# OCSYT/SoftwareRenderer

Measured on AMD Instinct MI355X. Metric: Mfragments/s (depth-tested + textured fragments, whole frame), higher is better.
Workload: dtype f32; 1 GPU; cfg3: 4096x4096, 1000000 triangles in 16 u16 meshes, 2048^2 RGBA8 nearest texture, program Dust2LambertFog, Back/LessEqual/Alpha; pipelining=1, parallelism=1 GPU

## Files before the change

### softwarerenderer_amd/csrc/swr_api.hip

```cpp
#include <hip/hip_runtime.h>
#include <hip/hiprtc.h>
#include <dlfcn.h>

#include <algorithm>
#include <cstddef>
#include <cmath>
#include <cstdio>
#include <cstdlib>
#include <cstring>
#include <map>
#include <memory>
#include <mutex>
#include <string>
#include <vector>
#if defined(SWR_RTC_FLAGS)
#include "swr_rtc_sources.inc"
#endif

#include "swr.h"
#include "swr_device.h"
#include "swr_geometry.hip.h"
#include "swr_binning.hip.h"
#include "swr_raster.hip.h"
#include "swr_raster_c.hip.h"
#include "swr_cull.hip.h"

using namespace swr;

#define SWR_STR2(x) #x
#define SWR_STR(x) SWR_STR2(x)

#include "swr_host.h"
#include "swr_rtc.h"
#include "swr_flush.h"

namespace {
int launch_flatten(swr_context* c, float* d_rgb, size_t n) {
    const int blocks = (int)std::min<size_t>((n + 255) / 256, 2048 * 8);
    hipLaunchKernelGGL(k_flatten_rgb, dim3(blocks), dim3(256), 0, c->stream, (const float4*)c->color, d_rgb, n);
    SWR_HIP(c, hipGetLastError());
    return SWR_OK;
}

int flatten_device(swr_context* c, float* d_rgb, bool validate) {
    if (!d_rgb) return fail(c, SWR_ERR_INVALID_ARG, "d_rgb is null");
    int rc = flush_locked(c); if (rc) return rc;
    const size_t n = band_pixels(c);
    if (!n) return SWR_OK;
    if (validate && (rc = sync_locked(c))) return rc;
    return launch_flatten(c, d_rgb, n);
}

int planes_transfer(swr_context* c, float* color, float* depth, bool to_host) {
    int rc = flush_and_sync_locked(c); if (rc) return rc;
    const size_t n = band_pixels(c);
    const hipMemcpyKind kind = to_host ? hipMemcpyDeviceToHost : hipMemcpyHostToDevice;
    if (n && color) SWR_HIP(c, hipMemcpyAsync(to_host ? (void*)color : c->color, to_host ? (void*)c->color : color, n * 16, kind, c->stream));
    if (n && depth) SWR_HIP(c, hipMemcpyAsync(to_host ? depth : c->depth, to_host ? c->depth : depth, n * 4, kind, c->stream));
    return sync_locked(c);
}

int pixel_transfer(swr_context* c, int x, int y, void* plane, size_t bytes, void* host, bool to_host) {
    if (x < 0 || x >= c->W || band_local_pixel_row(c, y) < 0) return SWR_OK;
    int rc = flush_and_sync_locked(c); if (rc) return rc;
    void* dev = static_cast<char*>(plane) + ((size_t)band_local_pixel_row(c, y) * c->W + x) * bytes;
    if (to_host) SWR_HIP(c, hipMemcpyAsync(host, dev, bytes, hipMemcpyDeviceToHost, c->stream));
    else SWR_HIP(c, hipMemcpyAsync(dev, host, bytes, hipMemcpyHostToDevice, c->stream));
    return sync_locked(c);
}
}

extern "C" {

int swr_abi_version(void) { return SWR_ABI_VERSION; }

#ifndef SWR_BUILD_HIPCC
#define SWR_BUILD_HIPCC "unknown"
#endif
#ifndef SWR_BUILD_SRC_SHA
#define SWR_BUILD_SRC_SHA "unknown"
#endif
#ifndef SWR_BUILD_EXTRA
#define SWR_BUILD_EXTRA ""
#endif
const char* swr_build_info(void) {
    return "hipcc=" SWR_BUILD_HIPCC "; csrc_sha256=" SWR_BUILD_SRC_SHA "; fma=" SWR_STR(SWR_NUMERICS_FMA) "; dot=" SWR_STR(SWR_DOT_PAIRWISE) "; extra=" SWR_BUILD_EXTRA;
}

int swr_numerics_mode(int* fma, int* dot_order) {
    if (!fma || !dot_order) return SWR_ERR_INVALID_ARG;
    *fma = SWR_NUMERICS_FMA; *dot_order = SWR_DOT_PAIRWISE;
    return SWR_OK;
}

int swr_set_transform_fma(swr_context* c, int transform_fused, int transform_normal_fused) {
    if (!c) return SWR_ERR_INVALID_ARG;
    std::lock_guard<std::mutex> lock_(c->mu);
    c->nm_flags = (transform_fused ? SWR_NM_TRANSFORM_FMA : 0u) | (transform_normal_fused ? SWR_NM_TRANSFORM_NORMAL_FMA : 0u);
    return SWR_OK;
}

int swr_get_transform_fma(swr_context* c, int* transform_fused, int* transform_normal_fused) {
    if (!c || !transform_fused || !transform_normal_fused) return SWR_ERR_INVALID_ARG;
    std::lock_guard<std::mutex> lock_(c->mu);
    *transform_fused = (c->nm_flags & SWR_NM_TRANSFORM_FMA) ? 1 : 0;
    *transform_normal_fused = (c->nm_flags & SWR_NM_TRANSFORM_NORMAL_FMA) ? 1 : 0;
    return SWR_OK;
}

const char* swr_last_error(const swr_context* ctx) { return ctx ? ctx->err.c_str() : g_create_error.c_str(); }

int swr_create(int device_id, swr_context** out) {
    if (!out) { g_create_error = "out is null"; return SWR_ERR_INVALID_ARG; }
    *out = nullptr;
    int n = 0;
    hipError_t e = hipGetDeviceCount(&n);
    if (e != hipSuccess || n <= 0) {
        g_create_error = std::string("no HIP device available: ") + hipGetErrorString(e) + " (this backend has no CPU fallback)";
        return SWR_ERR_NO_DEVICE;
    }
    if (device_id < 0 || device_id >= n) { g_create_error = "device id out of range"; return SWR_ERR_INVALID_ARG; }
    if ((e = hipSetDevice(device_id)) != hipSuccess) { g_create_error = hipGetErrorString(e); return SWR_ERR_HIP; }
    hipDeviceProp_t prop;
    if ((e = hipGetDeviceProperties(&prop, device_id)) != hipSuccess) { g_create_error = hipGetErrorString(e); return SWR_ERR_HIP; }
    if (strncmp(prop.gcnArchName, "gfx950", 6) != 0) {
        g_create_error = std::string("device is ") + prop.gcnArchName + "; libswr_hip.so carries gfx950 code objects only";
        return SWR_ERR_NO_DEVICE;
    }
    swr_context* c = new swr_context();
    c->device = device_id;
    snprintf(c->dev_name, sizeof c->dev_name, "%s (%s)", prop.name, prop.gcnArchName);
    if ((e = hipStreamCreateWithFlags(&c->own_stream, hipStreamNonBlocking)) != hipSuccess) {
        g_create_error = hipGetErrorString(e); delete c; return SWR_ERR_HIP;
    }
    c->stream = c->own_stream;
    if (ensure_front_stream(c)) { g_create_error = c->err; (void)hipStreamDestroy(c->own_stream); delete c; return SWR_ERR_HIP; }
    { const char* sf = getenv("SWR_SYNC_FLUSH"); c->sync_flush = sf && sf[0] == '1'; }
#ifdef SWR_TEST_HOOKS
    { const char* df = getenv("SWR_DEBUG_FILL_CAPACITY"); c->debug_fill_capacity = df ? (uint32_t)strtoul(df, nullptr, 10) : 0u; }
#endif
    int rc = ensure(c, c->d_counters, 65 * sizeof(Counters));
    if (!rc) rc = ensure(c, c->d_ctrl, 64);
    if (!rc && hipHostMalloc((void**)&c->host_poison, 64, hipHostMallocDefault) != hipSuccess) rc = SWR_ERR_OOM;
    if (!rc) { memset(c->host_poison, 0, 64); rc = reset_ctrl(c); }
    if (!rc) rc = ensure(c, c->d_total, 256 + 4096 * 8);
    if (!rc && hipMemsetAsync(c->d_total.p, 0, 256 + 4096 * 8, c->stream) != hipSuccess) rc = SWR_ERR_HIP;
    if (!rc && hipMemsetAsync(c->d_counters.p, 0, 65 * sizeof(Counters), c->stream) != hipSuccess) rc = SWR_ERR_HIP;
    if (rc) { g_create_error = c->err; swr_destroy(c); return rc; }
    *out = c;
    return SWR_OK;
}

void swr_destroy(swr_context* c) {
    if (!c) return;
    (void)hipSetDevice(c->device);
    (void)hipStreamSynchronize(c->stream);
    if (c->front_stream) (void)hipStreamSynchronize(c->front_stream);
    for (auto& d : c->draws) if (d.mesh && d.mesh->transient) c->garbage.push_back(d.mesh);
    for (auto& b : c->inflight) retire_batch(c, b);
    c->inflight.clear();
    collect_spans(c);
    free_garbage(c);
    c->draws.clear();
    c->progs.clear();
    for (swr_mesh* m : c->mesh_pool) destroy_mesh(m);
    c->mesh_pool.clear();
    for (hipEvent_t e : c->event_pool) (void)hipEventDestroy(e);
    for (auto& fs : c->slots) { if (fs.host) (void)hipHostFree(fs.host); if (fs.done) (void)hipEventDestroy(fs.done); }
    if (c->host_poison) (void)hipHostFree(c->host_poison);
    if (c->copy_stream) { (void)hipStreamSynchronize(c->copy_stream); (void)hipStreamDestroy(c->copy_stream); }
    for (int i = 0; i < 2; ++i) {
        if (c->present_flat[i]) (void)hipEventDestroy(c->present_flat[i]);
        if (c->present_done[i]) (void)hipEventDestroy(c->present_done[i]);
        release(c->present_buf[i]);
    }
    DevBuf* bufs[] = { &c->own_color, &c->own_depth, &c->d_slot_tb, &c->d_want, &c->d_ctrl, &c->d_pair_tile, &c->d_tile_list, &c->d_tile_stats,
                       &c->d_counters, &c->d_total, &c->d_scratch };
    for (DevBuf* b : bufs) release(*b);
    for (auto& s : c->sets) {
        DevBuf* sb[] = { &s.d_upload, &s.d_vout, &s.d_vnorm, &s.d_recs, &s.d_masks, &s.d_pcounts, &s.d_pair_refs, &s.d_tile_count, &s.d_tile_start, &s.d_order };
        for (DevBuf* b : sb) release(*b);
        if (s.front_done) (void)hipEventDestroy(s.front_done);
        if (s.raster_done) (void)hipEventDestroy(s.raster_done);
    }
    if (c->front_stream) (void)hipStreamDestroy(c->front_stream);
    if (c->f_tail_ev) (void)hipEventDestroy(c->f_tail_ev);
    if (c->r_front_ev) (void)hipEventDestroy(c->r_front_ev);
    if (c->own_stream) (void)hipStreamDestroy(c->own_stream);
    delete c;
}

#define SWR_ENTER(c)                                   \
    if (!(c)) return SWR_ERR_INVALID_ARG;              \
    std::lock_guard<std::mutex> lock_((c)->mu);        \
    (void)hipSetDevice((c)->device)

int swr_resize(swr_context* c, int width, int height) {
    SWR_ENTER(c);
    if (width > 65535 || height > 65535) return fail(c, SWR_ERR_INVALID_ARG, "render target larger than 65535");
    if (c->geometry_applied && width == c->W && height == c->H) return SWR_OK;
    int rc = flush_and_sync_locked(c); if (rc) return rc;
    c->W = width; c->H = height;
    c->geometry_applied = true;
    return apply_geometry(c);
}

int swr_set_band(swr_context* c, int first_tile_row, int n_tile_rows) {
    SWR_ENTER(c);
    const bool want_band = !(first_tile_row < 0 || n_tile_rows < 0);
    if (c->il_k == 0 && want_band == c->band_set && (!want_band || (first_tile_row == c->band_first && n_tile_rows == c->band_count)))
        return SWR_OK;
    int rc = flush_and_sync_locked(c); if (rc) return rc;
    c->il_k = 0; c->il_world = 1; c->il_rank = 0;
    c->band_set = want_band;
    if (want_band) { c->band_first = first_tile_row; c->band_count = n_tile_rows; }
    return apply_geometry(c);
}

int swr_set_band_interleaved(swr_context* c, int rank, int world, int stripe_tile_rows) {
    SWR_ENTER(c);
    if (world < 1 || rank < 0 || rank >= world || stripe_tile_rows < 1) return fail(c, SWR_ERR_INVALID_ARG, "bad interleaved band arguments");
    if (c->il_k == stripe_tile_rows && c->il_world == world && c->il_rank == rank) return SWR_OK;
    int rc = flush_and_sync_locked(c); if (rc) return rc;
    c->band_set = false;
    c->il_k = stripe_tile_rows; c->il_world = world; c->il_rank = rank;
    return apply_geometry(c);
}

int swr_bind_framebuffer(swr_context* c, void* color, void* depth) {
    SWR_ENTER(c);
    if ((color == nullptr) != (depth == nullptr)) return fail(c, SWR_ERR_INVALID_ARG, "bind both colour and depth, or neither");
    int rc = flush_locked(c); if (rc) return rc;
    if (!color && (rc = sync_locked(c))) return rc;
    c->ext_color = color; c->ext_depth = depth;
    return apply_geometry(c);
}

int swr_set_stream(swr_context* c, void* s) {
    SWR_ENTER(c);
    int rc = flush_and_sync_locked(c); if (rc) return rc;
    c->stream = s ? (hipStream_t)s : c->own_stream;
    return SWR_OK;
}

int swr_clear_color(swr_context* c, const float rgba[4]) {
    SWR_ENTER(c);
    if (!rgba) return fail(c, SWR_ERR_INVALID_ARG, "rgba is null");
    if (!c->draws.empty()) { int rc = flush_locked(c); if (rc) return rc; }
    memcpy(c->clear_rgba, rgba, 16);
    c->pend_clear_color = true;
    return SWR_OK;
}

int swr_clear_depth(swr_context* c) {
    SWR_ENTER(c);
    if (!c->draws.empty()) { int rc = flush_locked(c); if (rc) return rc; }
    c->pend_clear_depth = true;
    return SWR_OK;
}

int swr_flush(swr_context* c) { SWR_ENTER(c); return flush_locked(c); }

int swr_set_pipelining(swr_context* c, int mode) {
    SWR_ENTER(c);
    if (mode < 0 || mode > 2) return fail(c, SWR_ERR_INVALID_ARG, "pipelining mode must be 0 (off), 1 (every batch) or 2 (only frames of up to 2^15 tiles or batches of up to 2^17 triangles)");
    if (mode == c->pipelining) return SWR_OK;
    int rc = flush_and_sync_locked(c); if (rc) return rc;
    c->pipelining = mode;
    return ensure_front_stream(c);
}

int swr_get_pipelining(swr_context* c, int* mode) { SWR_ENTER(c); if (!mode) return SWR_ERR_INVALID_ARG; *mode = c->pipelining; return SWR_OK; }

int swr_sync(swr_context* c) {
    SWR_ENTER(c);
    return flush_and_sync_locked(c);
}

int swr_readback(swr_context* c, float* color, float* depth) { SWR_ENTER(c); return planes_transfer(c, color, depth, true); }

int swr_readback_rgb(swr_context* c, float* rgb) {
    SWR_ENTER(c);
    if (!rgb) return fail(c, SWR_ERR_INVALID_ARG, "rgb is null");
    int rc = flush_and_sync_locked(c); if (rc) return rc;
    size_t n = band_pixels(c);
    if (!n) return SWR_OK;
    if ((rc = ensure(c, c->d_scratch, n * 12))) return rc;
    if ((rc = launch_flatten(c, c->d_scratch.as<float>(), n))) return rc;
    SWR_HIP(c, hipMemcpyAsync(rgb, c->d_scratch.p, n * 12, hipMemcpyDeviceToHost, c->stream));
    return sync_locked(c);
}

int swr_present_rgb_async(swr_context* c, float* rgb, uint64_t* ticket) {
    SWR_ENTER(c);
    if (!rgb || !ticket) return fail(c, SWR_ERR_INVALID_ARG, "rgb or ticket is null");
    int rc = flush_locked(c); if (rc) return rc;
    const size_t n = band_pixels(c);
    const int slot = (int)(c->next_ticket & 1ull);
    if (!c->copy_stream) SWR_HIP(c, hipStreamCreateWithFlags(&c->copy_stream, hipStreamNonBlocking));
    for (int i = 0; i < 2; ++i) {
        if (!c->present_flat[i]) SWR_HIP(c, hipEventCreateWithFlags(&c->present_flat[i], hipEventDisableTiming));
        if (!c->present_done[i]) SWR_HIP(c, hipEventCreateWithFlags(&c->present_done[i], hipEventDisableTiming));
    }
    if (c->present_ticket[slot]) {
        SWR_HIP(c, hipEventSynchronize(c->present_done[slot]));
        bool stale = false;
        if ((rc = present_is_stale(c, slot, stale))) return rc;
        if (stale) c->stale_dropped[slot] = c->present_ticket[slot];
        c->present_ticket[slot] = 0;
    }
    if (n) {
        if (c->present_buf[slot].cap < n * 12) {
            SWR_HIP(c, hipStreamSynchronize(c->copy_stream));
            if ((rc = ensure(c, c->present_buf[slot], n * 12))) return rc;
        }
        if ((rc = launch_flatten(c, c->present_buf[slot].as<float>(), n))) return rc;
    }
    SWR_HIP(c, hipEventRecord(c->present_flat[slot], c->stream));
    SWR_HIP(c, hipStreamWaitEvent(c->copy_stream, c->present_flat[slot], 0));
    if (n) SWR_HIP(c, hipMemcpyAsync(rgb, c->present_buf[slot].p, n * 12, hipMemcpyDeviceToHost, c->copy_stream));
    SWR_HIP(c, hipEventRecord(c->present_done[slot], c->copy_stream));
    c->present_ticket[slot] = ++c->next_ticket;
    c->present_seq[slot] = c->next_seq - 1u;
    *ticket = c->present_ticket[slot];
    return SWR_OK;
}

int swr_present_wait(swr_context* c, uint64_t ticket) {
    SWR_ENTER(c);
    int slot = -1;
    for (int i = 0; i < 2; ++i) if (c->present_ticket[i] == ticket && ticket) slot = i;
    if (slot < 0) {
        if (!ticket || ticket > c->next_ticket) return fail(c, SWR_ERR_INVALID_ARG, "unknown present ticket");
        for (int i = 0; i < 2; ++i)
            if (c->stale_dropped[i] == ticket) { c->stale_dropped[i] = 0; return SWR_STALE; }
        return SWR_OK;
    }
    SWR_HIP(c, hipEventSynchronize(c->present_done[slot]));
    c->present_ticket[slot] = 0;
    bool stale = false;
    int rc = present_is_stale(c, slot, stale); if (rc) return rc;
    if (stale) {
        rc = sync_locked(c);
        return rc ? rc : SWR_STALE;
    }
    const uint32_t upto = c->present_seq[slot];
    size_t k = 0;
    while (k < c->inflight.size() && c->inflight[k].seq <= upto) { retire_batch(c, c->inflight[k], true); ++k; }
    c->inflight.erase(c->inflight.begin(), c->inflight.begin() + (std::ptrdiff_t)k);
    return SWR_OK;
}

int swr_host_register(swr_context* c, void* ptr, size_t bytes) {
    SWR_ENTER(c);
    if (!ptr || !bytes) return fail(c, SWR_ERR_INVALID_ARG, "null or empty host buffer");
    SWR_HIP(c, hipHostRegister(ptr, bytes, hipHostRegisterDefault));
    return SWR_OK;
}

int swr_host_unregister(swr_context* c, void* ptr) {
    SWR_ENTER(c);
    if (!ptr) return fail(c, SWR_ERR_INVALID_ARG, "null host buffer");
    int rc = flush_and_sync_locked(c); if (rc) return rc;
    SWR_HIP(c, hipHostUnregister(ptr));
    return SWR_OK;
}

int swr_flatten_rgb_device(swr_context* c, float* d_rgb) { SWR_ENTER(c); return flatten_device(c, d_rgb, true); }
int swr_flatten_rgb_device_async(swr_context* c, float* d_rgb) { SWR_ENTER(c); return flatten_device(c, d_rgb, false); }

int swr_replay_count(swr_context* c, uint64_t* out) { SWR_ENTER(c); if (!out) return SWR_ERR_INVALID_ARG; *out = c->replays; return SWR_OK; }
int swr_sync_count(swr_context* c, uint64_t* out) { SWR_ENTER(c); if (!out) return SWR_ERR_INVALID_ARG; *out = c->host_syncs; return SWR_OK; }

int swr_upload(swr_context* c, const float* color, const float* depth) {
    SWR_ENTER(c);
    return planes_transfer(c, const_cast<float*>(color), const_cast<float*>(depth), false);
}

int swr_color_device_ptr(swr_context* c, void** out) { SWR_ENTER(c); if (!out) return SWR_ERR_INVALID_ARG; *out = c->color; return SWR_OK; }
int swr_depth_device_ptr(swr_context* c, void** out) { SWR_ENTER(c); if (!out) return SWR_ERR_INVALID_ARG; *out = c->depth; return SWR_OK; }

int swr_get_pixel(swr_context* c, int x, int y, float rgba[4]) {
    SWR_ENTER(c);
    if (!rgba) return SWR_ERR_INVALID_ARG;
    rgba[0] = rgba[1] = rgba[2] = rgba[3] = 0.0f;
    return pixel_transfer(c, x, y, c->color, 16, rgba, true);
}
int swr_set_pixel(swr_context* c, int x, int y, const float rgba[4]) {
    SWR_ENTER(c);
    if (!rgba) return SWR_ERR_INVALID_ARG;
    return pixel_transfer(c, x, y, c->color, 16, const_cast<float*>(rgba), false);
}
int swr_get_depth(swr_context* c, int x, int y, float* d) {
    SWR_ENTER(c);
    if (!d) return SWR_ERR_INVALID_ARG;
    *d = SWR_FLOAT_MINVALUE;
    return pixel_transfer(c, x, y, c->depth, 4, d, true);
}
int swr_set_depth(swr_context* c, int x, int y, float d) {
    SWR_ENTER(c);
    return pixel_transfer(c, x, y, c->depth, 4, &d, false);
}

int swr_texture_create(swr_context* c, const uint8_t* rgba8, int w, int h, swr_texture** out) {
    SWR_ENTER(c);
    if (!rgba8 || w <= 0 || h <= 0 || !out) return fail(c, SWR_ERR_INVALID_ARG, "bad texture arguments");
    if ((uint64_t)w * (uint64_t)h >= (1ull << 30)) return fail(c, SWR_ERR_UNSUPPORTED, "textures of 2^30 texels or more are not supported (32-bit texel index)");
    swr_texture* t = new swr_texture();
    t->w = w; t->h = h;
    hipError_t e = hipMalloc((void**)&t->d_rgba, (size_t)w * h * 4);
    if (e == hipSuccess) e = hipMemcpyAsync(t->d_rgba, rgba8, (size_t)w * h * 4, hipMemcpyHostToDevice, c->stream);
    if (e != hipSuccess) {
        if (t->d_rgba) (void)hipFree(t->d_rgba);
        delete t;
        c->err = std::string("texture upload failed: ") + hipGetErrorString(e);
        return e == hipErrorOutOfMemory ? SWR_ERR_OOM : SWR_ERR_HIP;
    }
    *out = t;
    return SWR_OK;
}

int swr_texture_set_filter(swr_context* c, swr_texture* t, int bilinear) {
    SWR_ENTER(c);
    if (!t) return fail(c, SWR_ERR_INVALID_ARG, "texture is null");
    t->bilinear = bilinear != 0;
    if (t->bilinear && !t->d_blocked && (t->w & 3) == 0 && (t->h & 3) == 0) {
        SWR_HIP(c, hipMalloc((void**)&t->d_blocked, (size_t)t->w * t->h * 4));
        const int blocks = (int)std::min<size_t>(((size_t)t->w * t->h + 255) / 256, 2048 * 8);
        hipLaunchKernelGGL(k_block_texture, dim3(blocks), dim3(256), 0, c->stream, (const uint32_t*)t->d_rgba, (uint32_t*)t->d_blocked, t->w, t->h);
        SWR_HIP(c, hipGetLastError());
    }
    return SWR_OK;
}

int swr_texture_destroy(swr_context* c, swr_texture* t) {
    SWR_ENTER(c);
    if (!t) return SWR_OK;
    int rc = flush_and_sync_locked(c); if (rc) return rc;
    if (t->d_rgba) (void)hipFree(t->d_rgba);
    if (t->d_blocked) (void)hipFree(t->d_blocked);
    delete t;
    return SWR_OK;
}

int swr_texture_sample(swr_context* c, const swr_texture* t, const float* uv, int n, float* out) {
    SWR_ENTER(c);
    if (!t || !uv || !out || n < 0) return fail(c, SWR_ERR_INVALID_ARG, "bad texture_sample arguments");
    if (n == 0) return SWR_OK;
    const size_t off_out = ((size_t)n * 8 + 15) & ~(size_t)15;
    int rc = ensure(c, c->d_scratch, off_out + (size_t)n * 16);
    if (rc) return rc;
    float2* d_uv = c->d_scratch.as<float2>();
    float4* d_out = reinterpret_cast<float4*>(reinterpret_cast<char*>(c->d_scratch.p) + off_out);
    SWR_HIP(c, hipMemcpyAsync(d_uv, uv, (size_t)n * 8, hipMemcpyHostToDevice, c->stream));
    hipLaunchKernelGGL(k_texture_sample, dim3((n + 255) / 256), dim3(256), 0, c->stream, t->d_rgba, t->w, t->h, d_uv, n, d_out);
    SWR_HIP(c, hipGetLastError());
    SWR_HIP(c, hipMemcpyAsync(out, d_out, (size_t)n * 16, hipMemcpyDeviceToHost, c->stream));
    return sync_locked(c);
}

int swr_mesh_create(swr_context* c, const swr_vertex* v, int nv, const uint16_t* idx, int ni, swr_mesh** out) { SWR_ENTER(c); return make_mesh(c, v, nv, idx, ni, false, out); }

int swr_mesh_destroy(swr_context* c, swr_mesh* m) {
    SWR_ENTER(c);
    if (!m) return SWR_OK;
    int rc = flush_and_sync_locked(c); if (rc) return rc;
    destroy_mesh(m);
    return SWR_OK;
}

int swr_set_state(swr_context* c, float near_clip, float far_clip, int debug_mode) {
    SWR_ENTER(c);
    if (debug_mode != SWR_DEBUG_NONE && debug_mode != SWR_DEBUG_WIREFRAME) return fail(c, SWR_ERR_INVALID_ARG, "bad debug mode");
    if (!c->draws.empty() && (near_clip != c->near_clip || debug_mode != c->debug_mode)) {
        int rc = flush_locked(c); if (rc) return rc;
    }
    c->near_clip = near_clip; c->far_clip = far_clip; c->debug_mode = debug_mode;
    return SWR_OK;
}

int swr_initialize_tile_locks(swr_context* c, int width, int height) {
    SWR_ENTER(c);
    if (width <= 0 || height <= 0)
        return fail(c, SWR_ERR_INVALID_ARG, "Width and height must be positive non-zero values.");
    return SWR_OK;
}

int swr_render_mesh(swr_context* c, const swr_mesh* mesh, const float model[16], const float view[16], const float proj[16],
                    int program, const swr_uniforms* u, const swr_texture* tex, int cull, int depth_test, int blend) {
    SWR_ENTER(c); return record_draw(c, const_cast<swr_mesh*>(mesh), model, view, proj, program, u, tex, cull, depth_test, blend);
}

int swr_render_mesh_culled(swr_context* c, const swr_mesh* mesh, const float model[16], const float view[16], const float proj[16],
                           int program, const swr_uniforms* u, const swr_texture* tex, int cull, int depth_test, int blend) {
    SWR_ENTER(c); return record_draw(c, const_cast<swr_mesh*>(mesh), model, view, proj, program, u, tex, cull, depth_test, blend, true);
}

int swr_mesh_bounds(swr_context* c, const swr_mesh* mesh, float center_radius[4]) {
    SWR_ENTER(c);
    if (!mesh || !center_radius) return fail(c, SWR_ERR_INVALID_ARG, "bad mesh_bounds arguments");
    int rc = ensure_bounds(c, const_cast<swr_mesh*>(mesh));
    if (rc) return rc;
    SWR_HIP(c, hipMemcpyAsync(center_radius, mesh->d_bounds, 16, hipMemcpyDeviceToHost, use_front_stream(c)));
    SWR_HIP(c, hipStreamSynchronize(use_front_stream(c)));
    return SWR_OK;
}

int swr_is_sphere_in_frustum(swr_context* c, const float center_radius[4], const float model[16], const float view[16],
                             const float proj[16], int* inside) {
    SWR_ENTER(c);
    if (!center_radius || !model || !view || !proj || !inside) return fail(c, SWR_ERR_INVALID_ARG, "bad is_sphere_in_frustum arguments");
    int rc = ensure(c, c->d_scratch, 256);
    if (rc) return rc;
    float h[48];
    memcpy(h, model, 64); memcpy(h + 16, view, 64); memcpy(h + 32, proj, 64);
    char* base = reinterpret_cast<char*>(c->d_scratch.p);
    SWR_HIP(c, hipMemcpyAsync(base, h, sizeof h, hipMemcpyHostToDevice, c->stream));
    hipLaunchKernelGGL(k_frustum_test, dim3(1), dim3(64), 0, c->stream,
                       make_float4(center_radius[0], center_radius[1], center_radius[2], center_radius[3]),
                       (const float*)base, (uint32_t*)(base + 192), c->nm_flags);
    SWR_HIP(c, hipGetLastError());
    uint32_t r = 0;
    SWR_HIP(c, hipMemcpyAsync(&r, base + 192, 4, hipMemcpyDeviceToHost, c->stream));
    SWR_HIP(c, hipStreamSynchronize(c->stream));
    *inside = (int)r;
    return SWR_OK;
}

int swr_program_validate(const char* src, char* log, int log_len) { return swr_program_validate_vf(nullptr, src, log, log_len); }

int swr_program_validate_vf(const char* vertex_src, const char* src, char* log, int log_len) {
    if (!src) return SWR_ERR_INVALID_ARG;
    std::shared_ptr<const RtcCode> code;
    std::string msg;
    const int rc = rtc_compile(vertex_src, src, code, msg);
    if (log && log_len > 0) {
        const size_t n = std::min(msg.size(), (size_t)log_len - 1);
        memcpy(log, msg.data(), n); log[n] = '\0';
    }
    return rc;
}

int swr_program_create(swr_context* c, const char* src, int* program_id) { return swr_program_create_vf(c, nullptr, src, program_id); }

int swr_program_create_vf(swr_context* c, const char* vertex_src, const char* src, int* program_id) {
    SWR_ENTER(c);
    if (!src || !program_id) return fail(c, SWR_ERR_INVALID_ARG, "null argument to swr_program_create");
    std::shared_ptr<const RtcCode> code;
    std::string log;
    const int rc = rtc_compile(vertex_src, src, code, log);
    if (rc) { c->err = log; return rc; }
    auto p = std::make_shared<UserProg>();
    SWR_HIP(c, hipModuleLoadData(&p->mod, code->code.data()));
    for (int k = 0; k < 2; ++k) SWR_HIP(c, hipModuleGetFunction(&p->fn[k], p->mod, code->names[k].c_str()));
    if (code->has_vertex) {
        SWR_HIP(c, hipModuleGetFunction(&p->vertex_fn, p->mod, code->names[2].c_str()));
        SWR_HIP(c, hipModuleGetFunction(&p->setup_fn, p->mod, code->names[3].c_str()));
    }
    const int id = c->next_prog++;
    c->progs[id] = std::move(p);
    *program_id = id;
    return SWR_OK;
}

int swr_program_destroy(swr_context* c, int program_id) {
    SWR_ENTER(c);
    auto it = c->progs.find(program_id);
    if (it == c->progs.end()) return fail(c, SWR_ERR_INVALID_ARG, "unknown or destroyed user program id");
    c->progs.erase(it);
    return SWR_OK;
}

int swr_program_set_constants(swr_context* c, int program_id, const float* values, int n) {
    SWR_ENTER(c);
    auto it = c->progs.find(program_id);
    if (it == c->progs.end()) return fail(c, SWR_ERR_INVALID_ARG, "unknown or destroyed user program id");
    if (n < 0 || n > 64 || (n > 0 && !values)) return fail(c, SWR_ERR_INVALID_ARG, "between 0 and 64 constants");
    float* k = it->second->constants;
    for (int i = 0; i < 64; ++i) k[i] = i < n ? values[i] : 0.0f;
    return SWR_OK;
}

int swr_render_mesh_arrays(swr_context* c, const swr_vertex* v, int nv, const uint16_t* idx, int ni,
                           const float model[16], const float view[16], const float proj[16],
                           int program, const swr_uniforms* u, const swr_texture* tex, int cull, int depth_test, int blend) {
    SWR_ENTER(c);
    if (c->W <= 0 || c->H <= 0) return SWR_OK;
    swr_mesh* m = nullptr;
    int rc = make_mesh(c, v, nv, idx, ni, true, &m);
    if (rc) return rc;
    rc = record_draw(c, m, model, view, proj, program, u, tex, cull, depth_test, blend);
    if (rc || c->draws.empty() || c->draws.back().mesh != m) c->garbage.push_back(m);
    return rc;
}

int swr_interpolate(swr_context* c, const float* verts60, const float* w, int n, int interpolate, float* out) {
    SWR_ENTER(c);
    if (!verts60 || !w || !out || n < 0) return fail(c, SWR_ERR_INVALID_ARG, "bad interpolate arguments");
    if (n == 0) return SWR_OK;
    const size_t off_w = 256, off_o = 256 + (((size_t)n * 12 + 15) & ~(size_t)15);
    int rc = ensure(c, c->d_scratch, off_o + (size_t)n * 96);
    if (rc) return rc;
    char* base = reinterpret_cast<char*>(c->d_scratch.p);
    SWR_HIP(c, hipMemcpyAsync(base, verts60, 240, hipMemcpyHostToDevice, c->stream));
    SWR_HIP(c, hipMemcpyAsync(base + off_w, w, (size_t)n * 12, hipMemcpyHostToDevice, c->stream));
    hipLaunchKernelGGL(k_interpolate, dim3((n + 255) / 256), dim3(256), 0, c->stream,
                       (const float*)base, (const float*)(base + off_w), n, interpolate, (float*)(base + off_o));
    SWR_HIP(c, hipGetLastError());
    SWR_HIP(c, hipMemcpyAsync(out, base + off_o, (size_t)n * 96, hipMemcpyDeviceToHost, c->stream));
    return sync_locked(c);
}

int swr_get_stats(swr_context* c, swr_stats* out) {
    SWR_ENTER(c);
    if (!out) return SWR_ERR_INVALID_ARG;
    int rc = flush_and_sync_locked(c); if (rc) return rc;
    Counters host[65];
    unsigned long long frag[3] = { 0, 0, 0 };
    if (c->tile_stats_tiles) {
        unsigned long long* d3 = c->d_total.as<unsigned long long>() + 1;
        hipLaunchKernelGGL(k_reduce_tile_stats, dim3(1), dim3(1024), 0, c->stream, c->d_tile_stats.as<uint32_t>(),
                           (uint32_t)c->tile_stats_tiles, d3, 0);
        SWR_HIP(c, hipGetLastError());
        SWR_HIP(c, hipMemcpyAsync(frag, d3, 24, hipMemcpyDeviceToHost, c->stream));
    }
    unsigned long long carry[3] = { 0, 0, 0 };
    SWR_HIP(c, hipMemcpyAsync(carry, c->d_total.as<unsigned long long>() + 4, 24, hipMemcpyDeviceToHost, c->stream));
    SWR_HIP(c, hipMemcpyAsync(host, c->d_counters.p, sizeof host, hipMemcpyDeviceToHost, c->stream));
    if ((rc = sync_locked(c))) return rc;
    swr_stats s = {};
    for (int i = 0; i < 65; ++i) {
        s.triangles_in += host[i].triangles_in; s.triangles_setup += host[i].triangles_setup;
        s.triangles_clipped += host[i].triangles_clipped; s.tile_pairs += host[i].tile_pairs;
    }
    s.fragments_tested = frag[0] + carry[0]; s.fragments_shaded = frag[1] + carry[1]; s.fragments_written = frag[2] + carry[2];
    s.tile_pairs += c->host_tile_pairs;
    s.flushes = c->totals.flushes;
    *out = s;
    return SWR_OK;
}

int swr_reset_stats(swr_context* c) {
    SWR_ENTER(c);
    int rc = flush_locked(c); if (rc) return rc;
    SWR_HIP(c, hipMemsetAsync(c->d_counters.p, 0, 65 * sizeof(Counters), c->stream));
    if (c->tile_stats_tiles) SWR_HIP(c, hipMemsetAsync(c->d_tile_stats.p, 0, c->tile_stats_tiles * 12, c->stream));
    SWR_HIP(c, hipMemsetAsync(c->d_total.as<unsigned long long>() + 4, 0, 24, c->stream));
    c->totals = {}; c->host_tile_pairs = 0;
    return sync_locked(c);
}

int swr_profile_enable(swr_context* c, int on) {
    SWR_ENTER(c);
    int rc = flush_and_sync_locked(c); if (rc) return rc;
    c->profiling = on < 0 ? 0 : (on > 3 ? 1 : on);
    c->raster_span_no = 0;
    return SWR_OK;
}
int swr_profile_get(swr_context* c, swr_profile* out) {
    SWR_ENTER(c);
    if (!out) return SWR_ERR_INVALID_ARG;
    int rc = flush_and_sync_locked(c); if (rc) return rc;
    c->prof.flushes = c->totals.flushes;
    *out = c->prof;
    return SWR_OK;
}
int swr_profile_reset(swr_context* c) {
    SWR_ENTER(c);
    int rc = flush_and_sync_locked(c); if (rc) return rc;
    c->prof = {};
    c->raster_samples.clear();
    return SWR_OK;
}
int swr_profile_raster_samples(swr_context* c, float* out_ms, int capacity, int* n) {
    SWR_ENTER(c);
    if (!n || capacity < 0 || (capacity > 0 && !out_ms)) return SWR_ERR_INVALID_ARG;
    int rc = flush_and_sync_locked(c); if (rc) return rc;
    const int have = (int)c->raster_samples.size();
    for (int i = 0; i < std::min(have, capacity); ++i) out_ms[i] = c->raster_samples[(size_t)i];
    *n = have;
    return SWR_OK;
}

int swr_debug_counters(swr_context* c, uint64_t out[8]) {
    SWR_ENTER(c);
    if (!out) return SWR_ERR_INVALID_ARG;
    int rc = flush_and_sync_locked(c); if (rc) return rc;
    SWR_HIP(c, hipMemcpyAsync(out, c->d_total.as<unsigned long long>() + 8, 64, hipMemcpyDeviceToHost, c->stream));
    if ((rc = sync_locked(c))) return rc;
    SWR_HIP(c, hipMemsetAsync(c->d_total.as<unsigned long long>() + 8, 0, 64, c->stream));
    return SWR_OK;
}

int swr_selftest_division(swr_context* c, uint64_t samples, uint64_t seed, uint64_t out[8]) {
    SWR_ENTER(c);
    if (!out) return SWR_ERR_INVALID_ARG;
    int rc = flush_locked(c); if (rc) return rc;
    if ((rc = ensure(c, c->d_scratch, 64))) return rc;
    SWR_HIP(c, hipMemsetAsync(c->d_scratch.p, 0, 64, c->stream));
    const int iters = 1024;
    const uint64_t per_block = 256ull * (uint64_t)iters;
    const unsigned blocks = (unsigned)std::min<uint64_t>((samples + per_block - 1) / per_block, 1u << 20);
    if (blocks) hipLaunchKernelGGL(k_selftest_division, dim3(blocks), dim3(256), 0, c->stream, (unsigned long long)seed, iters,
                                   c->d_scratch.as<unsigned long long>());
    SWR_HIP(c, hipGetLastError());
    hipLaunchKernelGGL(k_selftest_recip, dim3(16384), dim3(256), 0, c->stream, c->d_scratch.as<unsigned long long>());
    SWR_HIP(c, hipGetLastError());
    SWR_HIP(c, hipMemcpyAsync(out, c->d_scratch.p, 64, hipMemcpyDeviceToHost, c->stream));
    return sync_locked(c);
}

int swr_device_name(swr_context* c, char* buf, int buflen) {
    SWR_ENTER(c);
    if (!buf || buflen <= 0) return SWR_ERR_INVALID_ARG;
    snprintf(buf, (size_t)buflen, "%s", c->dev_name);
    return SWR_OK;
}

}
```

### softwarerenderer_amd/csrc/swr_binning.hip.h

```cpp
#pragma once
#include "swr_device.h"

#define SWR_ORDER_BUCKETS 256

namespace swr {

struct BinArgs {
    const unsigned long long* __restrict__ slot_tb;
    const TriRec* __restrict__ recs;
    uint32_t odd_base;
    uint32_t slot_lo, slot_hi;
    uint32_t spt;
    int tiles_x;
    BandMap band;
    int width, height;
    uint32_t* __restrict__ tile_count;
    const uint32_t* __restrict__ tile_start;
    uint32_t* __restrict__ tile_list;
    uint32_t list_capacity;
    Counters* __restrict__ counters;
    Ctrl* __restrict__ ctrl;
    uint32_t seq;
    uint32_t replayable;
    const unsigned long long* __restrict__ total;
    const uint8_t* __restrict__ want;
    uint32_t tpw;
    uint32_t bin_blocks;
    int order_tiles_y;
    const uint8_t* __restrict__ tile_bucket;
    const uint32_t* __restrict__ order_hist;
    uint32_t* __restrict__ order_cursor;
    uint4* __restrict__ tile_order;
};


__device__ __forceinline__ void bin_overflow(const BinArgs& a) {
    a.counters->overflow = 1u;
    if (a.ctrl->host_flag) __hip_atomic_store(a.ctrl->host_flag + 1, 1u, __ATOMIC_RELAXED, __HIP_MEMORY_SCOPE_SYSTEM);
    if (a.replayable) {
        atomicMin(&a.ctrl->first_bad, a.seq);
        atomicMax(&a.ctrl->need, 2ull * (unsigned long long)a.list_capacity + 4096ull);
        __hip_atomic_store(&a.ctrl->poison, 1u, __ATOMIC_RELAXED, __HIP_MEMORY_SCOPE_AGENT);
        if (a.ctrl->host_flag) __hip_atomic_store(a.ctrl->host_flag, 1u, __ATOMIC_RELAXED, __HIP_MEMORY_SCOPE_SYSTEM);
    }
}

__device__ __forceinline__ uint32_t order_bucket(uint32_t w) {
    if (w == 0u) return 0u;
    const int e = 31 - __clz((int)w);
    const uint32_t m = e >= 3 ? ((w >> (e - 3)) & 7u) : ((w << (3 - e)) & 7u);
    return min((uint32_t)(e * 8) + m + 1u, (uint32_t)SWR_ORDER_BUCKETS - 1u);
}
__device__ __forceinline__ uint32_t tile_weight(uint32_t frags, uint32_t pairs) { return frags + 16u * pairs; }

__device__ __forceinline__ uint32_t order_tile_of_thread(uint32_t block, int tiles_x, int tiles_y) {
    const int sbx = (tiles_x + 15) >> 4;
    const int bx = (int)(block % (uint32_t)sbx), by = (int)(block / (uint32_t)sbx);
    const int t = threadIdx.x, q = t >> 6, w = t & 63;
    const int tx = bx * 16 + (q & 1) * 8 + (w & 7), ty = by * 16 + (q >> 1) * 8 + (w >> 3);
    return (tx < tiles_x && ty < tiles_y) ? (uint32_t)(ty * tiles_x + tx) : 0xffffffffu;
}
__host__ __device__ inline uint32_t order_blocks(int tiles_x, int tiles_y) { return (uint32_t)(((tiles_x + 15) / 16) * ((tiles_y + 15) / 16)); }

__device__ __forceinline__ void tile_place_block(const BinArgs& a, uint32_t block, uint32_t* s_suf, uint32_t* s_cnt) {
    const uint32_t t = threadIdx.x;
    s_suf[t] = a.order_hist[t];
    s_cnt[t] = 0u;
    __syncthreads();
    for (uint32_t off = 1; off < (uint32_t)SWR_ORDER_BUCKETS; off <<= 1) {
        const uint32_t v = t + off < (uint32_t)SWR_ORDER_BUCKETS ? s_suf[t + off] : 0u;
        __syncthreads();
        s_suf[t] += v;
        __syncthreads();
    }
    const uint32_t i = order_tile_of_thread(block, a.tiles_x, a.order_tiles_y);
    uint32_t b = 0, rank = 0;
    if (i != 0xffffffffu) {
        b = a.tile_bucket[i];
        rank = atomicAdd(&s_cnt[b], 1u);
    }
    __syncthreads();
    const uint32_t mine = s_cnt[t];
    __syncthreads();
    if (mine) s_cnt[t] = (s_suf[t] - a.order_hist[t]) + atomicAdd(&a.order_cursor[t], mine);
    __syncthreads();
    if (i != 0xffffffffu) {
        const uint32_t n_tiles = (uint32_t)(a.tiles_x * a.order_tiles_y);
        const uint32_t st = a.tile_start[i];
        const unsigned long long nxt = i + 1u < n_tiles ? (unsigned long long)a.tile_start[i + 1u] : *a.total;
        a.tile_order[s_cnt[b] + rank] = make_uint4(i, st, (uint32_t)(nxt - st), 0u);
    }
}

struct SlotData {
    int tminx, tminy, nx, ny;
    float sx[3], sy[3];
    int minX, maxX, minY, maxY;
    bool is_line;
};
__device__ __forceinline__ SlotData slot_load(const BinArgs& a, uint32_t slot, unsigned long long tb) {
    SlotData s;
    s.sx[0] = s.sx[1] = s.sx[2] = s.sy[0] = s.sy[1] = s.sy[2] = 0.f;
    s.minX = s.minY = 0; s.maxX = s.maxY = -1; s.is_line = false;
    SlotTiles st;
    slot_tiles(a.band, tb, st);
    s.tminx = st.tminx; s.tminy = st.tminy; s.nx = st.nx; s.ny = st.ny;
    if (s.nx * s.ny > SWR_SMALL_TILES) {
        const float4* __restrict__ rq = reinterpret_cast<const float4*>(a.recs + rec_index(slot, a.odd_base));
        const float4 r0 = rq[0], r1 = rq[1], r3 = rq[3];
        s.sx[0] = r0.x; s.sx[1] = r0.y; s.sx[2] = r0.z; s.sy[0] = r0.w; s.sy[1] = r1.x; s.sy[2] = r1.y;
        const uint32_t bbx = __float_as_uint(r3.y), bby = __float_as_uint(r3.z);
        s.minX = (int)(bbx & 0xffffu); s.maxX = (int)(bbx >> 16); s.minY = (int)(bby & 0xffffu); s.maxY = (int)(bby >> 16);
        s.is_line = (__float_as_uint(r3.w) & SWR_FLAG_LINE) != 0u;
    }
    return s;
}

template <bool FILL>
__device__ __forceinline__ void bin_big(const BinArgs& a, const SlotData& sd, uint32_t slot, bool big) {
    const int lane = threadIdx.x & 63;
    const int nt = sd.nx * sd.ny;
    unsigned long long med = __ballot(big && nt <= 64);
    while (med) {
        bool want[4];
        uint32_t tile[4], sslot[4], base[4];
#pragma unroll
        for (int j = 0; j < 4; ++j) {
            want[j] = false; tile[j] = 0u; sslot[j] = 0u; base[j] = 0u;
            if (med) {
                const int src = __ffsll((long long)med) - 1;
                med &= med - 1;
                const int s_tminx = __shfl(sd.tminx, src), s_tminy = __shfl(sd.tminy, src);
                const int s_nx = __shfl(sd.nx, src), s_nt = __shfl(nt, src);
                sslot[j] = (uint32_t)__shfl((int)slot, src);
                float bsx[3], bsy[3];
#pragma unroll
                for (int k = 0; k < 3; ++k) { bsx[k] = __shfl(sd.sx[k], src); bsy[k] = __shfl(sd.sy[k], src); }
                const int bminX = __shfl(sd.minX, src), bmaxX = __shfl(sd.maxX, src), bminY = __shfl(sd.minY, src), bmaxY = __shfl(sd.maxY, src);
                const bool b_line = __shfl((int)sd.is_line, src) != 0;
                if (lane < s_nt) {
                    const int ty = s_tminy + lane / s_nx, tx = s_tminx + lane % s_nx;
                    want[j] = band_local_row(a.band, ty) >= 0 && pair_may_cover(bsx, bsy, bminX, bmaxX, bminY, bmaxY, tx, ty, a.width, a.height, b_line);
                    tile[j] = (uint32_t)(band_local_row(a.band, ty) * a.tiles_x + tx);
                }
                if (want[j]) {
                    if (FILL) base[j] = atomicAdd(&a.tile_count[tile[j]], 1u);
                    else atomicAdd(&a.tile_count[tile[j]], 1u);
                }
            }
        }
        if (FILL) {
#pragma unroll
            for (int j = 0; j < 4; ++j) {
                if (want[j]) {
                    const uint32_t at = a.tile_start[tile[j]] + base[j];
                    if (at < a.list_capacity) a.tile_list[at] = sslot[j];
                    else bin_overflow(a);
                }
            }
        }
    }
    unsigned long long m = __ballot(big && nt > 64);
    while (m) {
        const int src = __ffsll((long long)m) - 1;
        m &= m - 1;
        const int s_tminx = __shfl(sd.tminx, src), s_tminy = __shfl(sd.tminy, src);
        const int s_nx = __shfl(sd.nx, src), s_nt = __shfl(nt, src);
        const uint32_t s_slot = (uint32_t)__shfl((int)slot, src);
        float bsx[3], bsy[3];
#pragma unroll
        for (int k = 0; k < 3; ++k) { bsx[k] = __shfl(sd.sx[k], src); bsy[k] = __shfl(sd.sy[k], src); }
        const int bminX = __shfl(sd.minX, src), bmaxX = __shfl(sd.maxX, src), bminY = __shfl(sd.minY, src), bmaxY = __shfl(sd.maxY, src);
        const bool b_line = __shfl((int)sd.is_line, src) != 0;
        for (int i0 = 0; i0 < s_nt; i0 += 64) {
            const int i = i0 + lane;
            bool want = i < s_nt;
            int ty = 0, tx = 0;
            if (want) {
                ty = s_tminy + i / s_nx; tx = s_tminx + i % s_nx;
                want = band_local_row(a.band, ty) >= 0 && pair_may_cover(bsx, bsy, bminX, bmaxX, bminY, bmaxY, tx, ty, a.width, a.height, b_line);
            }
            if (want) {
                const uint32_t tile = (uint32_t)(band_local_row(a.band, ty) * a.tiles_x + tx);
                if (FILL) {
                    const uint32_t at = a.tile_start[tile] + atomicAdd(&a.tile_count[tile], 1u);
                    if (at < a.list_capacity) a.tile_list[at] = s_slot;
                    else bin_overflow(a);
                } else {
                    atomicAdd(&a.tile_count[tile], 1u);
                }
            }
        }
    }
}

#define SWR_BIN_TABLE_LOG2 8
#define SWR_BIN_TABLE (1 << SWR_BIN_TABLE_LOG2)
template <bool FILL>
__device__ __forceinline__ void bin_block_slots(const BinArgs& a, uint32_t slot, unsigned long long tb, uint32_t want_in, uint32_t* s_key, uint32_t* s_val) {
    const SlotData sd = slot_load(a, slot, tb);
    const int nt = sd.nx * sd.ny;
    const bool big = nt > SWR_SMALL_TILES;
    const int nt_small = big ? 0 : nt;
    if (!__syncthreads_or(nt != 0)) return;
    for (int e = threadIdx.x; e < SWR_BIN_TABLE; e += 256) { s_key[e] = 0u; s_val[e] = 0u; }
    __syncthreads();
    uint32_t packed[SWR_SMALL_TILES];
    SlotTiles st; st.tminx = sd.tminx; st.tminy = sd.tminy; st.nx = sd.nx; st.ny = sd.ny;
    SmallTileWalk w(st);
    const uint32_t wmask = nt_small ? want_in : 0u;
#pragma unroll
    for (int i = 0; i < SWR_SMALL_TILES; ++i) {
        packed[i] = 0u;
        if (i < nt_small) {
            if ((wmask >> i) & 1u) {
                const uint32_t tile = (uint32_t)(band_local_row(a.band, w.ty) * a.tiles_x + w.tx);
                uint32_t e = (tile * 0x9E3779B1u) >> (32 - SWR_BIN_TABLE_LOG2);
                bool placed = false;
                for (int probe = 0; probe < 16; ++probe) {
                    const uint32_t prev = atomicCAS(&s_key[e], 0u, tile + 1u);
                    if (prev == 0u || prev == tile + 1u) { placed = true; break; }
                    e = (e + 1u) & (SWR_BIN_TABLE - 1u);
                }
                if (placed) {
                    const uint32_t rank = atomicAdd(&s_val[e], 1u);
                    packed[i] = e | (rank << 12) | 0x80000000u;
                } else if (FILL) {
                    const uint32_t at = a.tile_start[tile] + atomicAdd(&a.tile_count[tile], 1u);
                    if (at < a.list_capacity) a.tile_list[at] = slot;
                    else bin_overflow(a);
                } else {
                    atomicAdd(&a.tile_count[tile], 1u);
                }
            }
            w.next();
        }
    }
    __syncthreads();
    for (int e = threadIdx.x; e < SWR_BIN_TABLE; e += 256) {
        const uint32_t key = s_key[e];
        if (key) {
            const uint32_t tile = key - 1u, n = s_val[e];
            if (FILL) s_val[e] = a.tile_start[tile] + atomicAdd(&a.tile_count[tile], n);
            else atomicAdd(&a.tile_count[tile], n);
        }
    }
    if (FILL) {
        __syncthreads();
#pragma unroll
        for (int i = 0; i < SWR_SMALL_TILES; ++i) {
            if (packed[i] & 0x80000000u) {
                const uint32_t at = s_val[packed[i] & 0xfffu] + ((packed[i] >> 12) & 0x7ffffu);
                if (at < a.list_capacity) a.tile_list[at] = slot;
                else bin_overflow(a);
            }
        }
    }
    bin_big<FILL>(a, sd, slot, big);
}

template <bool FILL>
__global__ __launch_bounds__(256) void k_bin(BinArgs a) {
    SWR_FRONT_ENTER();
    __shared__ uint32_t s_key[SWR_BIN_TABLE];
    __shared__ uint32_t s_val[SWR_BIN_TABLE];
    if (FILL && batch_poisoned(a.ctrl, a.seq)) return;
    if (FILL && blockIdx.x >= a.bin_blocks) {
        static_assert(SWR_BIN_TABLE >= SWR_ORDER_BUCKETS, "tile_place_block borrows the hash table's LDS");
        tile_place_block(a, blockIdx.x - a.bin_blocks, s_key, s_val);
        return;
    }
    const uint32_t wave_id = (blockIdx.x * 256u + threadIdx.x) >> 6, lane_id = threadIdx.x & 63u;
    const bool has_tri = lane_id < a.tpw;
    const uint32_t first = a.slot_lo + (wave_id * a.tpw + lane_id) * a.spt;
    auto in_round = [&](uint32_t si) { return has_tri && si < a.spt && first + si < a.slot_hi; };
    auto tb_of = [&](uint32_t si) { return in_round(si) ? a.slot_tb[first + si] : SWR_TB_INVALID; };
    auto want_of = [&](uint32_t si) { return in_round(si) ? (uint32_t)a.want[first + si] : 0u; };
    unsigned long long tb = tb_of(0);
    uint32_t wm = want_of(0);
    for (uint32_t si = 0; si < a.spt; ++si) {
        const unsigned long long tb_next = tb_of(si + 1);
        const uint32_t wm_next = want_of(si + 1);
        bin_block_slots<FILL>(a, first + si, tb, wm, s_key, s_val);
        tb = tb_next; wm = wm_next;
    }
}

#define SWR_SCAN_BLOCK 256
__device__ __forceinline__ unsigned long long block_sum(unsigned long long v, unsigned long long* s_part) {
#pragma unroll
    for (int off = 32; off > 0; off >>= 1) {
        unsigned lo = (unsigned)v, hi = (unsigned)(v >> 32);
        v += ((unsigned long long)(unsigned)__shfl_xor((int)hi, off) << 32) | (unsigned)__shfl_xor((int)lo, off);
    }
    if ((threadIdx.x & 63u) == 0u) s_part[threadIdx.x >> 6] = v;
    __syncthreads();
    unsigned long long t = 0;
    for (int w = 0; w < SWR_SCAN_BLOCK / 64; ++w) t += s_part[w];
    return t;
}

__global__ __launch_bounds__(SWR_SCAN_BLOCK) void k_scan_sums(const uint32_t* __restrict__ count, uint32_t n,
                                                    unsigned long long* __restrict__ sums) {
    SWR_FRONT_ENTER();
    __shared__ unsigned long long s_part[SWR_SCAN_BLOCK / 64];
    const uint32_t i = blockIdx.x * (uint32_t)SWR_SCAN_BLOCK + threadIdx.x;
    const unsigned long long t = block_sum(i < n ? count[i] : 0u, s_part);
    if (threadIdx.x == 0) sums[blockIdx.x] = t;
}

__global__ __launch_bounds__(SWR_SCAN_BLOCK) void k_scan_apply(uint32_t* __restrict__ count, uint32_t* __restrict__ start,
                                                     uint32_t n, const unsigned long long* __restrict__ sums,
                                                     unsigned long long* __restrict__ total_out,
                                                     unsigned long long capacity, uint32_t seq, Ctrl* __restrict__ ctrl,
                                                     Counters* __restrict__ counters, int poison_on_overflow,
                                                     const uint32_t* __restrict__ tile_work, uint32_t* __restrict__ order_hist,
                                                     uint8_t* __restrict__ tile_bucket) {
    SWR_FRONT_ENTER();
    __shared__ unsigned long long s_part[SWR_SCAN_BLOCK / 64];
    __shared__ unsigned long long s_wave[SWR_SCAN_BLOCK / 64];
    __shared__ uint32_t s_oh[SWR_ORDER_BUCKETS];
    static_assert(SWR_ORDER_BUCKETS <= SWR_SCAN_BLOCK, "one thread per bucket clears / flushes the block's histogram");
    const uint32_t tid = threadIdx.x, lane = tid & 63u, wv = tid >> 6;
    if (tid < (uint32_t)SWR_ORDER_BUCKETS) s_oh[tid] = 0u;
    unsigned long long mine = 0ull;
    for (uint32_t j = tid; j < blockIdx.x; j += (uint32_t)SWR_SCAN_BLOCK) mine += sums[j];
    const unsigned long long off = block_sum(mine, s_part);
    const uint32_t i = blockIdx.x * (uint32_t)SWR_SCAN_BLOCK + tid;
    const uint32_t c = i < n ? count[i] : 0u;
    if (i < n) {
        const uint32_t ob = order_bucket(tile_weight(tile_work[i], c));
        tile_bucket[i] = (uint8_t)ob;
        atomicAdd(&s_oh[ob], 1u);
    }
    unsigned long long incl = c;
#pragma unroll
    for (int o = 1; o < 64; o <<= 1) {
        unsigned lo = (unsigned)incl, hi = (unsigned)(incl >> 32);
        unsigned long long v = ((unsigned long long)(unsigned)__shfl_up((int)hi, o) << 32) | (unsigned)__shfl_up((int)lo, o);
        if (lane >= (uint32_t)o) incl += v;
    }
    if (lane == 63u) s_wave[wv] = incl;
    __syncthreads();
    if (tid < (uint32_t)SWR_ORDER_BUCKETS && s_oh[tid]) atomicAdd(&order_hist[tid], s_oh[tid]);
    unsigned long long wave_off = 0;
    for (uint32_t w = 0; w < wv; ++w) wave_off += s_wave[w];
    const unsigned long long excl = off + wave_off + incl - c;
    if (i < n) {
        start[i] = (uint32_t)min(excl, 0xffffffffull);
        count[i] = 0u;
    }
    if (blockIdx.x == gridDim.x - 1 && tid == (uint32_t)SWR_SCAN_BLOCK - 1u) {
        const unsigned long long total = excl + c;
        *total_out = total;
        if (total > capacity) {
            if (!poison_on_overflow) return;
            atomicMin(&ctrl->first_bad, seq);
            atomicMax(&ctrl->need, total);
            __hip_atomic_store(&ctrl->poison, 1u, __ATOMIC_RELAXED, __HIP_MEMORY_SCOPE_AGENT);
            if (ctrl->host_flag) __hip_atomic_store(ctrl->host_flag, 1u, __ATOMIC_RELAXED, __HIP_MEMORY_SCOPE_SYSTEM);
        } else if (poison_on_overflow && !batch_poisoned(ctrl, seq)) {
            atomicAdd(&counters->tile_pairs, total);
        }
    }
}

#define SWR_SORT_LDS 2048

__device__ __forceinline__ void cmpx_lds(uint32_t* s, uint32_t i, uint32_t p, uint32_t n) {
    if (p < n) {
        uint32_t a = s[i], b = s[p];
        if (a > b) { s[i] = b; s[p] = a; }
    }
}
__device__ __forceinline__ void cmpx_glb(uint32_t* g, uint32_t i, uint32_t p, uint32_t n) {
    if (p < n) {
        uint32_t a = g[i], b = g[p];
        if (a > b) { g[i] = b; g[p] = a; }
    }
}

#define SWR_SORT_TPB 1
#define SWR_SORT_TPW 4
#define SWR_SORT_WAVE_SYNC() do { __builtin_amdgcn_fence(__ATOMIC_ACQ_REL, "workgroup"); __builtin_amdgcn_wave_barrier(); } while (0)
__device__ __forceinline__ void sort_tile(uint32_t n, uint32_t start, uint32_t* __restrict__ tile_list, uint32_t tile,
                                          uint32_t* __restrict__ pair_tile, uint32_t* s_keys, uint32_t key_in) {
    if (n == 0) return;
    const uint32_t lane = threadIdx.x & 63u;
    for (uint32_t i = lane; i < n; i += 64) pair_tile[start + i] = tile;
    if (n < 2) return;
    uint32_t* seg = tile_list + start;

    if (n <= 64) {
        uint32_t key = lane < n ? key_in : 0xffffffffu;
#define SWR_CMPX(other_expr, lower_cond) { const uint32_t other = (uint32_t)(other_expr); \
                                            key = (lower_cond) ? min(key, other) : max(key, other); }
#define SWR_DPP(ctrl) __builtin_amdgcn_update_dpp(0, (int)key, ctrl, 0xf, 0xf, false)
#define SWR_XOR1  SWR_CMPX(SWR_DPP(0xB1), (lane & 1u) == 0u)
#define SWR_XOR2  SWR_CMPX(SWR_DPP(0x4E), (lane & 2u) == 0u)
#define SWR_XOR4  { const int up = SWR_DPP(0x124), dn = SWR_DPP(0x12C);               \
                    SWR_CMPX((lane & 4u) ? up : dn, (lane & 4u) == 0u) }
#define SWR_XOR8  SWR_CMPX(SWR_DPP(0x128), (lane & 8u) == 0u)
#define SWR_XOR16 SWR_CMPX(__shfl((int)key, (int)(lane ^ 16u)), (lane & 16u) == 0u)
        SWR_XOR1
        SWR_CMPX(SWR_DPP(0x1B), (lane & 2u) == 0u) SWR_XOR1
        SWR_CMPX(SWR_DPP(0x141), (lane & 4u) == 0u) SWR_XOR2 SWR_XOR1
        SWR_CMPX(SWR_DPP(0x140), (lane & 8u) == 0u) SWR_XOR4 SWR_XOR2 SWR_XOR1
        SWR_CMPX(__shfl((int)key, (int)(lane ^ 31u)), (lane & 16u) == 0u) SWR_XOR8 SWR_XOR4 SWR_XOR2 SWR_XOR1
        SWR_CMPX(__shfl((int)key, (int)(lane ^ 63u)), (lane & 32u) == 0u) SWR_XOR16 SWR_XOR8 SWR_XOR4 SWR_XOR2 SWR_XOR1
#undef SWR_XOR16
#undef SWR_XOR8
#undef SWR_XOR4
#undef SWR_XOR2
#undef SWR_XOR1
#undef SWR_DPP
#undef SWR_CMPX
        if (lane < n) seg[lane] = key;
        return;
    }

    uint32_t m = 1;
    while (m < n) m <<= 1;
    const bool in_lds = n <= SWR_SORT_LDS;
    uint32_t* buf = in_lds ? s_keys : seg;
    if (in_lds) {
        for (uint32_t i = lane; i < n; i += 64) s_keys[i] = seg[i];
        SWR_SORT_WAVE_SYNC();
    }
    for (uint32_t k = 2; k <= m; k <<= 1) {
        for (uint32_t t = lane; t < (m >> 1); t += 64) {
            uint32_t blk = t / (k >> 1), off = t % (k >> 1);
            uint32_t i = blk * k + off, p = blk * k + (k - 1 - off);
            if (i < n) { if (in_lds) cmpx_lds(buf, i, p, n); else cmpx_glb(buf, i, p, n); }
        }
        SWR_SORT_WAVE_SYNC();
        for (uint32_t j = k >> 2; j > 0; j >>= 1) {
            for (uint32_t t = lane; t < (m >> 1); t += 64) {
                uint32_t i = 2 * j * (t / j) + (t % j), p = i + j;
                if (i < n) { if (in_lds) cmpx_lds(buf, i, p, n); else cmpx_glb(buf, i, p, n); }
            }
            SWR_SORT_WAVE_SYNC();
        }
    }
    if (in_lds) {
        for (uint32_t i = lane; i < n; i += 64) seg[i] = s_keys[i];
    }
}

__global__ __launch_bounds__(64 * SWR_SORT_TPB) void k_sort_tiles(const uint32_t* __restrict__ tile_start,
                                                   const uint32_t* __restrict__ tile_count,
                                                   uint32_t* __restrict__ tile_list, uint32_t n_tiles,
                                                   uint32_t* __restrict__ pair_tile, const Ctrl* __restrict__ ctrl, uint32_t seq,
                                                   const uint4* __restrict__ tile_order ) {
    SWR_FRONT_ENTER();
    __shared__ uint32_t s_keys_all[SWR_SORT_TPB][SWR_SORT_LDS];
    static_assert(sizeof(s_keys_all) <= SWR_FRONT_MAX_LDS, "k_sort_tiles must fit beside the raster kernel (swr_device.h)");
    if (batch_poisoned(ctrl, seq)) return;
    static_assert(SWR_SORT_TPW <= 64, "one lane per tile of the wave fetches its count and start");
    const uint32_t first = (blockIdx.x * SWR_SORT_TPB + (threadIdx.x >> 6)) * SWR_SORT_TPW;
    const uint32_t lane = threadIdx.x & 63u;
    const uint32_t waves = gridDim.x * SWR_SORT_TPB, entry = (first / SWR_SORT_TPW) + lane * waves;
    const bool mine = lane < SWR_SORT_TPW && entry < n_tiles;
    const uint4 desc_l = mine ? tile_order[entry] : make_uint4(0u, 0u, 0u, 0u);
    const uint32_t tile_l = desc_l.x;
    const uint32_t cnt_l = desc_l.z, st_l = desc_l.y;
    uint32_t keys[SWR_SORT_TPW];
#pragma unroll
    for (int t = 0; t < SWR_SORT_TPW; ++t) {
        const uint32_t n = (uint32_t)__builtin_amdgcn_readlane((int)cnt_l, t), start = (uint32_t)__builtin_amdgcn_readlane((int)st_l, t);
        keys[t] = (lane < n && n <= 64u) ? tile_list[start + lane] : 0xffffffffu;
    }
#pragma unroll
    for (int t = 0; t < SWR_SORT_TPW; ++t) {
        const uint32_t n = (uint32_t)__builtin_amdgcn_readlane((int)cnt_l, t), start = (uint32_t)__builtin_amdgcn_readlane((int)st_l, t);
        sort_tile(n, start, tile_list, (uint32_t)__builtin_amdgcn_readlane((int)tile_l, t), pair_tile, s_keys_all[threadIdx.x >> 6], keys[t]);
        SWR_SORT_WAVE_SYNC();
    }
}

}
```

### softwarerenderer_amd/csrc/swr_flush.h

```cpp
#pragma once
#include "swr_raster_select.h"

namespace {
int kernel_class(int program) { return program == SWR_PROG_DEBUG_VARYINGS || program >= SWR_PROG_USER_BASE ? program : 0; }

void destroy_mesh(swr_mesh* m) {
    if (m->d_verts) (void)hipFree(m->d_verts);
    if (m->d_idx) (void)hipFree(m->d_idx);
    if (m->d_bounds) (void)hipFree(m->d_bounds);
    delete m;
}
const size_t kMeshPoolBytes = (size_t)1 << 30;
void trim_mesh_pool(swr_context* c) {
    while (c->mesh_pool_bytes > kMeshPoolBytes && !c->mesh_pool.empty()) {
        swr_mesh* m = c->mesh_pool.front();
        c->mesh_pool.erase(c->mesh_pool.begin());
        c->mesh_pool_bytes -= m->cap_verts + m->cap_idx;
        destroy_mesh(m);
    }
}
void pool_mesh(swr_context* c, swr_mesh* m) {
    c->mesh_pool.push_back(m);
    c->mesh_pool_bytes += m->cap_verts + m->cap_idx;
    if (c->mesh_pool_bytes > 2 * kMeshPoolBytes) trim_mesh_pool(c);
}
void free_garbage(swr_context* c) {
    for (swr_mesh* m : c->garbage) pool_mesh(c, m);
    c->garbage.clear();
    c->prog_garbage.clear();
    trim_mesh_pool(c);
}

int validate_locked(swr_context* c);

int drain_streams(swr_context* c) {
    SWR_HIP(c, hipStreamSynchronize(c->stream));
    if (c->front_stream) SWR_HIP(c, hipStreamSynchronize(c->front_stream));
    for (auto& s : c->sets) s.raster_pending = false;
    c->f_tail_pending = c->r_front_pending = false;
    return SWR_OK;
}

int sync_locked(swr_context* c) {
    ++c->host_syncs;
    int rc = drain_streams(c);
    if (rc) return rc;
    rc = validate_locked(c);
    collect_spans(c);
    free_garbage(c);
    for (auto& fs : c->slots) fs.busy = false;
    return rc;
}

enum { MODE_SYNC = 0, MODE_ASYNC = 1 };
struct UploadLayout { size_t off_vb, off_tb, off_bp, off_vis, off_consts, bytes; };
static UploadLayout upload_layout(size_t nd, size_t v_blocks, size_t t_blocks, bool any_cull, bool user) {
    const auto r256 = [](size_t x) { return (x + 255) & ~(size_t)255; };
    UploadLayout u;
    u.off_vb = r256(nd * sizeof(DrawParams));
    u.off_tb = r256(u.off_vb + v_blocks * sizeof(BlockMap));
    u.off_bp = r256(u.off_tb + t_blocks * sizeof(BlockMap));
    u.off_vis = r256(u.off_bp + (any_cull ? nd * sizeof(void*) : 0));
    const size_t vis_end = u.off_vis + (any_cull ? nd * 4 : 0);
    u.off_consts = r256(vis_end);
    u.bytes = user ? u.off_consts + nd * 64 * sizeof(float) : vis_end;
    return u;
}
template <class T> T* at(void* base, size_t off) { return reinterpret_cast<T*>(static_cast<char*>(base) + off); }

struct OrderView { uint4* tile_order; uint32_t* tile_work; uint32_t* hist; uint32_t* cursor; uint8_t* tile_bucket; };
static size_t order_bytes(uint32_t n_tiles) { return (size_t)n_tiles * (sizeof(uint4) + 4 + 1 + 4) + 2 * SWR_ORDER_BUCKETS * 4; }
static OrderView order_view(RasterSet& S, uint32_t n_tiles) {
    uint4* order = S.d_order.as<uint4>();
    uint32_t* work = reinterpret_cast<uint32_t*>(order + n_tiles), *hist = work + n_tiles, *cursor = hist + SWR_ORDER_BUCKETS;
    return { order, work, hist, cursor, reinterpret_cast<uint8_t*>(cursor + SWR_ORDER_BUCKETS) };
}

struct Pass {
    const Batch& b;
    RasterSet& S;
    hipStream_t F;
    int mode;
    bool cc, cd;
    UploadLayout up = {};
    uint32_t odd_base = 0;
};

static bool b_needs_vnorm(const Batch& b) { return !b.draws.empty() && kernel_class(b.draws[0].p.program) != 0; }
static bool b_has_user_program(const Batch& b) { return !b.draws.empty() && b.draws[0].p.program >= SWR_PROG_USER_BASE; }
static bool b_has_user_vertex(const Batch& b) { return b_has_user_program(b) && b.draws[0].prog && b.draws[0].prog->vertex_fn; }
#ifndef SWR_DENSE_RECORDS
#define SWR_DENSE_RECORDS 1
#endif
const unsigned long long kMaxPairs = 1ull << 30;

size_t pair_capacity(const swr_context* c) {
    size_t cap = std::min(c->d_tile_list.cap / 4, c->d_pair_tile.cap / 4);
    for (int i = 0; i < (c->pipelining ? 2 : 1); ++i) {
        const RasterSet& s = c->sets[i];
        cap = std::min(cap, std::min(std::min(s.d_masks.cap / 32, s.d_pcounts.cap / 8), s.d_pair_refs.cap / 16));
    }
    return cap;
}
int ensure_pairs(swr_context* c, size_t n) {
    int rc;
    if ((rc = ensure(c, c->d_tile_list, n * 4))) return rc;
    if ((rc = ensure(c, c->d_pair_tile, n * 4))) return rc;
    for (int i = 0; i < (c->pipelining ? 2 : 1); ++i) {
        RasterSet& s = c->sets[i];
        if ((rc = ensure(c, s.d_masks, n * 32))) return rc;
        if ((rc = ensure(c, s.d_pair_refs, n * 16))) return rc;
        if ((rc = ensure(c, s.d_pcounts, n * 8 + 64))) return rc;
    }
    return SWR_OK;
}

int run_clear(swr_context* c, const Batch& b, bool& cc, bool& cd) {
    size_t n = band_pixels(c);
    if (n && (cc || cd)) {
        ScopedSpan sp(c, ST_CLEAR);
        int blocks = (int)std::min<size_t>((n + 255) / 256, 2048 * 8);
        float4 rgba = make_float4(b.clear_rgba[0], b.clear_rgba[1], b.clear_rgba[2], b.clear_rgba[3]);
        hipLaunchKernelGGL(k_clear, dim3(blocks), dim3(256), 0, c->stream, b.color, b.depth, n, rgba,
                           cc ? 1 : 0, cd ? 1 : 0, (const Ctrl*)c->d_ctrl.as<Ctrl>(), b.seq);
        SWR_HIP(c, hipGetLastError());
    }
    cc = cd = false;
    return SWR_OK;
}

int launch_raster(swr_context* c, Pass& P, uint32_t n_tiles);

int bin_and_raster(swr_context* c, Pass& P, uint32_t lo, uint32_t hi, bool counts_clear = false) {
    const uint32_t n_tiles = (uint32_t)c->tiles_x * (uint32_t)c->band_tile_rows;
    if (n_tiles == 0 || lo >= hi) return SWR_OK;
    int rc;
    const Batch& b = P.b; RasterSet& S = P.S;
    const hipStream_t F = P.F; const int mode = P.mode;
    const Ctrl* ctrl = c->d_ctrl.as<Ctrl>();
    unsigned long long* d_total = c->d_total.as<unsigned long long>();
    const OrderView ov = order_view(S, n_tiles);
    BinArgs ba;
    ba.slot_tb = c->d_slot_tb.as<unsigned long long>();
    ba.recs = S.d_recs.as<TriRec>();
    ba.odd_base = P.odd_base;
    ba.slot_lo = lo; ba.slot_hi = hi;
    ba.spt = b.wireframe ? 6u : 2u;
    ba.width = c->W; ba.height = c->H;
    ba.tiles_x = c->tiles_x;
    ba.band = host_band_map(c);
    ba.tile_count = S.d_tile_count.as<uint32_t>();
    ba.tile_start = S.d_tile_start.as<uint32_t>();
    ba.tile_list = c->d_tile_list.as<uint32_t>();
    ba.list_capacity = (uint32_t)std::min<size_t>(pair_capacity(c), 0xffffffffu);
    ba.counters = c->d_counters.as<Counters>();
    ba.ctrl = c->d_ctrl.as<Ctrl>();
    ba.seq = b.seq; ba.replayable = mode == MODE_ASYNC ? 1u : 0u;
    ba.total = c->d_total.as<unsigned long long>();
    ba.want = c->d_want.as<uint8_t>();
    const uint32_t bin_threads = (hi - lo + ba.spt - 1u) / ba.spt;
    ba.tpw = 64u;
    while (ba.tpw > 4u && bin_threads < ba.tpw * 1024u) ba.tpw >>= 1;
    const uint32_t bin_blocks = (bin_threads + 4u * ba.tpw - 1u) / (4u * ba.tpw);
    {
        ScopedSpan sp(c, ST_BIN, F);
        if (!counts_clear) {
            SWR_HIP(c, hipMemsetAsync(ba.tile_count, 0, (size_t)n_tiles * 4, F));
            SWR_HIP(c, hipMemsetAsync(ov.hist, 0, 2 * SWR_ORDER_BUCKETS * 4, F));
        }
        hipLaunchKernelGGL(k_bin<false>, dim3(bin_blocks), dim3(256), 0, F, ba);
        const unsigned scan_blocks = (n_tiles + (unsigned)SWR_SCAN_BLOCK - 1u) / (unsigned)SWR_SCAN_BLOCK;
        unsigned long long* sums = d_total + 32;
        hipLaunchKernelGGL(k_scan_sums, dim3(scan_blocks), dim3(SWR_SCAN_BLOCK), 0, F, (const uint32_t*)ba.tile_count, n_tiles, sums);
        const unsigned long long cap = mode == MODE_ASYNC ? (unsigned long long)ba.list_capacity : ~0ull;
        hipLaunchKernelGGL(k_scan_apply, dim3(scan_blocks), dim3(SWR_SCAN_BLOCK), 0, F, ba.tile_count,
                           S.d_tile_start.as<uint32_t>(), n_tiles, (const unsigned long long*)sums, d_total,
                           cap, b.seq, c->d_ctrl.as<Ctrl>(), c->d_counters.as<Counters>() + 64,
                           mode == MODE_ASYNC ? 1 : 0, (const uint32_t*)ov.tile_work, ov.hist, ov.tile_bucket);
        SWR_HIP(c, hipGetLastError());
    }
    uint32_t cover_items = ba.list_capacity;
    if (mode == MODE_SYNC) {
        unsigned long long total = 0;
        SWR_HIP(c, hipMemcpyAsync(&total, d_total, 8, hipMemcpyDeviceToHost, F));
        SWR_HIP(c, hipStreamSynchronize(F));
        if (total > kMaxPairs && hi - lo > 2) {
            uint32_t mid = lo + (((hi - lo) / 2u) & ~1u);
            if (mid == lo) mid = lo + 2;
            if ((rc = bin_and_raster(c, P, lo, mid))) return rc;
            return bin_and_raster(c, P, mid, hi);
        }
        if (total == 0) return run_clear(c, b, P.cc, P.cd);
        if (total > 0xffffffffull) return fail(c, SWR_ERR_UNSUPPORTED, "a single triangle covers more tile pairs than one round can hold");
        c->host_tile_pairs += total;
        if ((rc = ensure_pairs(c, (size_t)std::min<unsigned long long>(total + total / 4 + 4096, std::max(total, kMaxPairs))))) return rc;
        ba.tile_list = c->d_tile_list.as<uint32_t>();
        ba.list_capacity = (uint32_t)std::min<size_t>(pair_capacity(c), 0xffffffffu);
        cover_items = (uint32_t)total;
    }
    {
        ScopedSpan sp(c, ST_BIN, F);
        BinArgs bf = ba;
        if (mode == MODE_ASYNC && c->debug_fill_capacity) bf.list_capacity = std::min(bf.list_capacity, c->debug_fill_capacity);
        bf.bin_blocks = bin_blocks;
        bf.order_tiles_y = c->band_tile_rows;
        bf.tile_bucket = ov.tile_bucket; bf.order_hist = ov.hist; bf.order_cursor = ov.cursor; bf.tile_order = ov.tile_order;
        hipLaunchKernelGGL(k_bin<true>, dim3(bin_blocks + order_blocks(c->tiles_x, c->band_tile_rows)), dim3(256), 0, F, bf);
        SWR_HIP(c, hipGetLastError());
    }
    {
        ScopedSpan sp(c, ST_SORT, F);
        hipLaunchKernelGGL(k_sort_tiles, dim3((n_tiles + SWR_SORT_TPB * SWR_SORT_TPW - 1u) / (SWR_SORT_TPB * SWR_SORT_TPW)), dim3(64 * SWR_SORT_TPB), 0, F, S.d_tile_start.as<uint32_t>(),
                           S.d_tile_count.as<uint32_t>(), c->d_tile_list.as<uint32_t>(), n_tiles, c->d_pair_tile.as<uint32_t>(), ctrl, b.seq,
                           (const uint4*)ov.tile_order);
        SWR_HIP(c, hipGetLastError());
    }
    if (cover_items) {
        ScopedSpan sp(c, ST_COVER, F);
        CoverArgs ca;
        ca.recs = S.d_recs.as<TriRec>();
        ca.odd_base = P.odd_base;
        ca.tile_list = c->d_tile_list.as<uint32_t>();
        ca.pair_tile = c->d_pair_tile.as<uint32_t>();
        ca.masks = S.d_masks.as<uint4>();
        ca.info = S.d_pcounts.as<uint2>();
        ca.refs = S.d_pair_refs.as<uint4>();
        ca.n_pairs = d_total;
        ca.ctrl = ctrl; ca.seq = b.seq;
        ca.fp = frame_params(c, b.near_clip);
        ca.dbg = d_total + 8;
        const dim3 cg((unsigned)((((cover_items + (uint32_t)SWR_COVER_BLOCK - 1u) / (uint32_t)SWR_COVER_BLOCK) + 7u) & ~7u)), cb(SWR_COVER_BLOCK);
        if (b.wireframe) hipLaunchKernelGGL(k_cover<true>, cg, cb, 0, F, ca);
        else hipLaunchKernelGGL(k_cover<false>, cg, cb, 0, F, ca);
        SWR_HIP(c, hipGetLastError());
    }
    if (F != c->stream) {
        SWR_HIP(c, hipEventRecord(S.front_done, F));
        SWR_HIP(c, hipStreamWaitEvent(c->stream, S.front_done, 0));
    } else if (c->pipelining && mode == MODE_ASYNC) {
        SWR_HIP(c, hipEventRecord(c->r_front_ev, c->stream));
        c->r_front_pending = true;
    }
    if ((rc = launch_raster(c, P, n_tiles))) return rc;
    if (c->pipelining && S.raster_done) {
        SWR_HIP(c, hipEventRecord(S.raster_done, c->stream));
        S.raster_pending = true;
    }
    return SWR_OK;
}

int launch_raster(swr_context* c, Pass& P, uint32_t n_tiles) {
    const Batch& b = P.b; RasterSet& S = P.S;
    const OrderView ov = order_view(S, n_tiles);
    ScopedSpan sp(c, ST_RASTER);
    RasterArgs ra;
    ra.fp = frame_params(c, b.near_clip);
    ra.recs = S.d_recs.as<TriRec>();
    ra.vout = S.d_vout.as<VOut>();
    ra.vout_bytes = (uint32_t)std::min<size_t>(S.d_vout.cap, 0xfffffff0u);
    ra.vnorm = b_needs_vnorm(b) ? S.d_vnorm.as<float4>() : nullptr;
    ra.user_consts = b_has_user_program(b) ? at<const float>(S.d_upload.p, P.up.off_consts) : nullptr;
    ra.draws = at<const DrawParams>(S.d_upload.p, 0);
    ra.tile_start = S.d_tile_start.as<uint32_t>();
    ra.tile_count = S.d_tile_count.as<uint32_t>();
    ra.pair_refs = S.d_pair_refs.as<uint4>();
    ra.color = b.color; ra.depth = b.depth;
    ra.tile_stats = c->d_tile_stats.as<uint32_t>();
    memcpy(ra.clear_rgba, b.clear_rgba, 16);
    ra.clear_color_on = P.cc ? 1 : 0;
    ra.clear_depth_on = P.cd ? 1 : 0;
    ra.tile_order = ov.tile_order;
    ra.tile_work = ov.tile_work;
    ra.n_tiles = n_tiles;
    ra.dbg = c->d_total.as<unsigned long long>() + 8;
    ra.ctrl = c->d_ctrl.as<Ctrl>(); ra.seq = b.seq;
    RasterTraits traits;
    traits.wireframe = b.wireframe;
    for (auto& d : b.draws) traits.add(d.p.program, d.p.blend, d.p.depth_test);
    ra.depth_only_grows = traits.depth_only_grows ? 1 : 0;
    const RasterKernel kernel = select_raster_kernel(traits);
    using RasterFn = void (*)(RasterArgs, const uint4*, const uint2*);
    static const RasterFn table[] = {
        k_raster_c<false, true, SWR_PROG_DEBUG_VARYINGS, -1, -1, true>,
        k_raster_c<false, true, SWR_PROG_DEBUG_VARYINGS>,
        k_raster_c<true, true>,
        k_raster_c<false, true, -1, -1, -1, true>,
        k_raster_c<false, true, SWR_PROG_PHONG_4POINT, SWR_BLEND_ALPHA, SWR_DEPTH_LESSEQUAL>,
        k_raster_c<false, true>,
        k_raster_c<false, false, SWR_PROG_DUST2_LAMBERT_FOG, SWR_BLEND_ALPHA, SWR_DEPTH_LESSEQUAL>,
        k_raster_c<false, false, SWR_PROG_GOURAUD, SWR_BLEND_ALPHA, SWR_DEPTH_LESSEQUAL>,
        k_raster_c<false, false>,
    };
    static_assert(sizeof table / sizeof table[0] == (size_t)RasterKernel::user, "one kernel per built-in RasterKernel, in its order");
    const dim3 g((n_tiles + 511u) & ~511u), t(64);
    const uint4* mk = (const uint4*)S.d_masks.as<uint4>();
    const uint2* pc = (const uint2*)S.d_pcounts.as<uint2>();
    if (kernel == RasterKernel::user || kernel == RasterKernel::user_none) {
        void* args[] = { &ra, &mk, &pc };
        hipFunction_t fn = b.draws[0].prog->fn[kernel == RasterKernel::user_none ? 1 : 0];
        SWR_HIP(c, hipModuleLaunchKernel(fn, g.x, 1, 1, t.x, 1, 1, 0, c->stream, args, nullptr));
    } else {
        hipLaunchKernelGGL(table[(int)kernel], g, t, 0, c->stream, ra, mk, pc);
    }
    SWR_HIP(c, hipGetLastError());
    P.cc = P.cd = false;
    return SWR_OK;
}

struct BatchGeometry {
    std::vector<DrawParams> hp;
    std::vector<BlockMap> vblocks, tblocks;
    uint64_t V = 0, T = 0; bool any_cull = false;
};
static BatchGeometry batch_geometry(const Batch& b) {
    BatchGeometry g;
    const size_t nd = b.draws.size();
    g.hp.resize(nd);
    std::vector<uint32_t> frag_reps;
    for (size_t i = 0; i < nd; ++i) {
        DrawParams p = b.draws[i].p;
        p.vert_base = (uint32_t)g.V; p.tri_base = (uint32_t)g.T;
        for (uint32_t f = 0; f < p.n_verts; f += SWR_GEOM_BLOCK) g.vblocks.push_back({ (uint32_t)i, f });
        for (uint32_t f = 0; f < p.n_tris; f += SWR_GEOM_BLOCK) g.tblocks.push_back({ (uint32_t)i, f });
        g.V += p.n_verts; g.T += p.n_tris;
        g.any_cull = g.any_cull || b.draws[i].frustum_cull;
        p.frag_draw = (uint32_t)i;
        for (uint32_t j : frag_reps) {
            const DrawParams& q = g.hp[j];
            if (q.program == p.program && q.blend == p.blend && q.depth_test == p.depth_test && q.tex == p.tex && q.tex_w == p.tex_w &&
                q.tex_h == p.tex_h && memcmp(&q.u, &p.u, sizeof p.u) == 0 &&
                (p.program < SWR_PROG_USER_BASE || *b.draws[j].uconsts == *b.draws[i].uconsts)) { p.frag_draw = j; break; }
        }
        if (p.frag_draw == (uint32_t)i && p.n_verts > 0 && !b.draws[i].frustum_cull && frag_reps.size() < 64) frag_reps.push_back((uint32_t)i);
        g.hp[i] = p;
    }
    return g;
}

int launch_geometry(swr_context* c, const Pass& P, const BatchGeometry& g, uint32_t n_tiles, int count_stats) {
    const Batch& b = P.b; RasterSet& S = P.S; const hipStream_t F = P.F;
    const UserProg* vprog = b_has_user_vertex(b) ? b.draws[0].prog.get() : nullptr;
    const auto launch = [&](hipFunction_t user_fn, const void* builtin, size_t blocks, void** args) {
        return user_fn ? hipModuleLaunchKernel(user_fn, (unsigned)blocks, 1, 1, SWR_GEOM_BLOCK, 1, 1, 0, F, args, nullptr)
                       : hipLaunchKernel(builtin, dim3((unsigned)blocks), dim3(SWR_GEOM_BLOCK), args, 0, F);
    };
    const uint32_t nd = (uint32_t)b.draws.size();
    const DrawParams* d_draws = at<const DrawParams>(S.d_upload.p, 0);
    const BlockMap* d_vblocks = at<const BlockMap>(S.d_upload.p, P.up.off_vb);
    const BlockMap* d_tblocks = at<const BlockMap>(S.d_upload.p, P.up.off_tb);
    const uint32_t* d_visible = nullptr;
    if (g.any_cull) {
        ScopedSpan sp(c, ST_VERTEX, F);
        uint32_t* vis = at<uint32_t>(S.d_upload.p, P.up.off_vis);
        hipLaunchKernelGGL(k_frustum_cull, dim3((nd + 63) / 64), dim3(64), 0, F, d_draws,
                           at<const float4* const>(S.d_upload.p, P.up.off_bp), nd, vis);
        SWR_HIP(c, hipGetLastError());
        d_visible = vis;
    }
    float4* a_vnorm = b_needs_vnorm(b) ? S.d_vnorm.as<float4>() : (float4*)nullptr;
    if (!g.vblocks.empty()) {
        ScopedSpan sp(c, ST_VERTEX, F);
        VOut* a_vout = S.d_vout.as<VOut>();
        float* a_fog = at<float>(S.d_upload.p, offsetof(DrawParams, fog_r1));
        uint32_t* a_zero = S.d_tile_count.as<uint32_t>();
        uint32_t a_n_zero = n_tiles;
        uint32_t* a_hist = order_view(S, n_tiles).hist;
        const float* a_consts = at<const float>(S.d_upload.p, P.up.off_consts);
        void* args[] = { &d_draws, &d_vblocks, &a_vout, &d_visible, &a_fog, &a_vnorm, &a_zero, &a_n_zero, &a_hist, &a_consts };
        SWR_HIP(c, launch(vprog ? vprog->vertex_fn : nullptr, (const void*)k_vertex, g.vblocks.size(), args));
    }
    {
        ScopedSpan sp(c, ST_SETUP, F);
        FrameParams fp = frame_params(c, b.near_clip);
        const VOut* a_vout = S.d_vout.as<VOut>();
        VOut* a_pool = S.d_vout.as<VOut>() + g.V;
        uint32_t a_pool_base = (uint32_t)g.V;
        TriRec* a_recs = S.d_recs.as<TriRec>();
        uint32_t a_odd_base = P.odd_base;
        unsigned long long* a_tb = c->d_slot_tb.as<unsigned long long>();
        uint8_t* a_want = c->d_want.as<uint8_t>();
        Counters* a_counters = c->d_counters.as<Counters>();
        const Ctrl* a_ctrl = c->d_ctrl.as<Ctrl>();
        uint32_t a_seq = b.seq;
        int a_count = count_stats, a_wire = b.wireframe ? 1 : 0;
        void* args[] = { &d_draws, &d_tblocks, &a_vout, &a_pool, &a_pool_base, &a_recs, &a_odd_base, &a_tb, &a_want, &fp, &a_counters, &a_ctrl, &a_seq,
                         &a_count, &a_wire, &d_visible, &a_vnorm };
        SWR_HIP(c, launch(vprog ? vprog->setup_fn : nullptr, (const void*)k_setup, g.tblocks.size(), args));
    }
    return SWR_OK;
}

int execute_batch(swr_context* c, const Batch& b, int mode, int count_stats) {
    bool cc = b.clear_color, cd = b.clear_depth;
    if (b.draws.empty()) return run_clear(c, b, cc, cd);
    int rc;
    if ((rc = ensure_front_stream(c))) return rc;
    const BatchGeometry g = batch_geometry(b);
    const uint64_t V = g.V, T = g.T;
    const uint32_t n_tiles = (uint32_t)c->tiles_x * (uint32_t)c->band_tile_rows;
    const bool piped = mode == MODE_ASYNC && (c->pipelining == 1 || (c->pipelining == 2 && (T <= c->pipeline_max_tris ||
                                                                                            n_tiles <= c->pipeline_max_tiles)));
    Pass P{ b, c->sets[c->pipelining ? (b.seq & 1u) : 0u], piped ? c->front_stream : c->stream, mode, cc, cd };
    RasterSet& S = P.S; const hipStream_t F = P.F;
    if (c->pipelining && mode != MODE_ASYNC) SWR_HIP(c, hipStreamSynchronize(c->front_stream));
    if (c->pipelining && mode == MODE_ASYNC) {
        if (!piped && c->f_tail_pending) {
            SWR_HIP(c, hipEventRecord(c->f_tail_ev, c->front_stream));
            SWR_HIP(c, hipStreamWaitEvent(c->stream, c->f_tail_ev, 0));
            c->f_tail_pending = false;
        }
        if (piped && c->r_front_pending) {
            SWR_HIP(c, hipStreamWaitEvent(c->front_stream, c->r_front_ev, 0));
            c->r_front_pending = false;
        }
        if (piped) c->f_tail_pending = true;
    }
    const uint64_t spt = b.wireframe ? 6 : 2;
    if (V + 4 * T >= (1ull << 26) || spt * T >= 0xffffffffull)
        return fail(c, SWR_ERR_UNSUPPORTED, "internal error: a batch beyond 2^26 vertex-stage records reached execute_batch (record_draw flushes before)");
    if (T == 0) return run_clear(c, b, cc, cd);
    if (n_tiles > (1u << 20))
        return fail(c, SWR_ERR_UNSUPPORTED, "more than 2^20 tiles in one band (a target beyond 16384 x 16384): render it in tile-row bands (swr_set_band)");

    P.up = upload_layout(b.draws.size(), g.vblocks.size(), g.tblocks.size(), g.any_cull, b_has_user_program(b));
    if ((rc = ensure(c, S.d_upload, P.up.bytes))) return rc;
    if ((rc = ensure(c, S.d_vout, (size_t)(V + 4 * T) * sizeof(VOut)))) return rc;
    if (b_needs_vnorm(b) && (rc = ensure(c, S.d_vnorm, S.d_vout.cap / 4))) return rc;
    P.odd_base = (b.wireframe || !SWR_DENSE_RECORDS) ? 0u : record_odd_base(T);
    if ((rc = ensure(c, S.d_recs, (size_t)(spt * T + 2) * sizeof(TriRec)))) return rc;
    if ((rc = ensure(c, c->d_slot_tb, (size_t)(spt * T) * 8))) return rc;
    if ((rc = ensure(c, c->d_want, (size_t)(spt * T) + 64))) return rc;
    if ((rc = ensure(c, S.d_tile_count, (size_t)n_tiles * 4))) return rc;
    if ((rc = ensure(c, S.d_tile_start, (size_t)n_tiles * 4))) return rc;
    if ((rc = ensure(c, S.d_order, order_bytes(n_tiles)))) return rc;
    if (c->tile_stats_tiles != n_tiles) {
        if (c->tile_stats_tiles) {
            hipLaunchKernelGGL(k_reduce_tile_stats, dim3(1), dim3(1024), 0, c->stream, c->d_tile_stats.as<uint32_t>(),
                               (uint32_t)c->tile_stats_tiles, c->d_total.as<unsigned long long>() + 4, 1);
            SWR_HIP(c, hipGetLastError());
        }
        if ((rc = ensure(c, c->d_tile_stats, (size_t)n_tiles * 12))) return rc;
        SWR_HIP(c, hipMemsetAsync(c->d_tile_stats.p, 0, (size_t)n_tiles * 12, c->stream));
        c->tile_stats_tiles = n_tiles;
    }
    if (piped && S.raster_pending) SWR_HIP(c, hipStreamWaitEvent(F, S.raster_done, 0));
    if (S.hist_tiles != n_tiles) {
        SWR_HIP(c, hipMemsetAsync(order_view(S, n_tiles).tile_work, 0, (size_t)n_tiles * 4, F));
        S.hist_tiles = n_tiles;
    }
    const size_t nd = b.draws.size();
    char* stage = (char*)slot_acquire(c, P.up.bytes);
    if (!stage) return fail(c, SWR_ERR_OOM, "hipHostMalloc failed for the upload staging block");
    memcpy(stage, g.hp.data(), nd * sizeof(DrawParams));
    if (!g.vblocks.empty()) memcpy(stage + P.up.off_vb, g.vblocks.data(), g.vblocks.size() * sizeof(BlockMap));
    memcpy(stage + P.up.off_tb, g.tblocks.data(), g.tblocks.size() * sizeof(BlockMap));
    if (g.any_cull) {
        const float4** bp = at<const float4*>(stage, P.up.off_bp);
        for (size_t i = 0; i < nd; ++i) bp[i] = b.draws[i].frustum_cull ? b.draws[i].mesh->d_bounds : nullptr;
    }
    if (b_has_user_program(b)) {
        float* uc = at<float>(stage, P.up.off_consts);
        for (size_t i = 0; i < nd; ++i) memcpy(uc + 64 * i, b.draws[i].uconsts->data(), 64 * sizeof(float));
    }
    SWR_HIP(c, hipMemcpyAsync(S.d_upload.p, stage, P.up.bytes, hipMemcpyHostToDevice, F));
    if ((rc = launch_geometry(c, P, g, n_tiles, count_stats))) return rc;
    const bool counts_clear = !g.vblocks.empty() && n_tiles != 0;
    rc = bin_and_raster(c, P, 0, (uint32_t)(spt * T), counts_clear);
    slot_submit(c);
    if (rc) return rc;
    if (c->pipelining && mode != MODE_ASYNC) SWR_HIP(c, hipStreamSynchronize(c->stream));
    if (P.cc || P.cd) return run_clear(c, b, P.cc, P.cd);
    return SWR_OK;
}

void retire_batch(swr_context* c, Batch& b, bool complete = false) {
    for (auto& d : b.draws) {
        if (d.mesh && d.mesh->transient) { if (complete) pool_mesh(c, d.mesh); else c->garbage.push_back(d.mesh); }
        if (d.prog && !complete) c->prog_garbage.push_back(std::move(d.prog));
    }
    b.draws.clear();
}

int check_list_overflow(swr_context* c) {
    if (!c->host_poison || !((volatile uint32_t*)c->host_poison)[1]) return SWR_OK;
    c->host_poison[1] = 0;
    return fail(c, SWR_ERR_HIP, "internal error: a (triangle, tile) pair did not fit its tile list and was dropped (Counters::overflow)");
}

int reset_ctrl(swr_context* c) {
    Ctrl fresh; fresh.poison = 0; fresh.first_bad = 0xffffffffu; fresh.need = 0; fresh.host_flag = c->host_poison;
    SWR_HIP(c, hipMemcpy(c->d_ctrl.p, &fresh, sizeof fresh, hipMemcpyHostToDevice));
    return SWR_OK;
}

int validate_locked(swr_context* c) {
    if (c->inflight.empty()) return check_list_overflow(c);
    int rc = SWR_OK;
    if (*(volatile uint32_t*)c->host_poison) {
        Ctrl h;
        SWR_HIP(c, hipMemcpy(&h, c->d_ctrl.p, sizeof h, hipMemcpyDeviceToHost));
        *c->host_poison = 0;
        c->host_poison[1] = 0;
        if ((rc = reset_ctrl(c))) return rc;
        std::vector<Batch> todo;
        todo.swap(c->inflight);
        c->replays++;
        for (auto& b : todo) {
            if (!rc && b.seq >= h.first_bad) {
                rc = execute_batch(c, b, MODE_SYNC, b.seq != h.first_bad);
                retire_batch(c, b);
            } else {
                retire_batch(c, b, true);
            }
        }
        if (!rc) rc = drain_streams(c);
        if (!rc) rc = check_list_overflow(c);
        return rc;
    }
    for (auto& b : c->inflight) retire_batch(c, b, true);
    c->inflight.clear();
    return check_list_overflow(c);
}

int flush_locked(swr_context* c) {
    if (c->W <= 0 || c->H <= 0 || band_pixels(c) == 0) {
        for (auto& d : c->draws) if (d.mesh && d.mesh->transient) c->garbage.push_back(d.mesh);
        c->draws.clear(); c->pend_verts = c->pend_tris = 0;
        c->pend_clear_color = c->pend_clear_depth = false;
        return SWR_OK;
    }
    if (c->draws.empty() && !c->pend_clear_color && !c->pend_clear_depth) return SWR_OK;
    Batch b;
    b.draws.swap(c->draws);
    b.clear_color = c->pend_clear_color; b.clear_depth = c->pend_clear_depth;
    memcpy(b.clear_rgba, c->clear_rgba, 16);
    b.near_clip = c->near_clip;
    b.wireframe = c->debug_mode == SWR_DEBUG_WIREFRAME;
    if (b.wireframe && b_needs_vnorm(b)) {
        for (auto& d : b.draws) if (d.mesh && d.mesh->transient) c->garbage.push_back(d.mesh);
        c->pend_verts = c->pend_tris = 0;
        return fail(c, SWR_ERR_UNSUPPORTED, b_has_user_program(b) ? "user programs are not available in DebugMode.Wireframe"
                                                                   : "SWR_PROG_DEBUG_VARYINGS is not available in DebugMode.Wireframe");
    }
    b.seq = c->next_seq++;
    b.color = c->color; b.depth = c->depth;
    c->pend_clear_color = c->pend_clear_depth = false;
    c->pend_verts = c->pend_tris = 0;
    if (!b.draws.empty()) c->totals.flushes++;
    const bool optimistic = !c->sync_flush && pair_capacity(c) > 0;
    int rc = execute_batch(c, b, optimistic ? MODE_ASYNC : MODE_SYNC, 1);
    if (optimistic && !rc) {
        c->inflight.push_back(std::move(b));
        if (c->inflight.size() >= 64) {
            if ((rc = drain_streams(c))) return rc;
            rc = validate_locked(c);
        }
    } else {
        retire_batch(c, b);
    }
    return rc;
}

int flush_and_sync_locked(swr_context* c) {
    int rc = flush_locked(c);
    return rc ? rc : sync_locked(c);
}

int ensure_bounds(swr_context* c, swr_mesh* m) {
    if (m->bounds_ready) return SWR_OK;
    if (!m->d_bounds) SWR_HIP(c, hipMalloc((void**)&m->d_bounds, sizeof(float4)));
    hipLaunchKernelGGL(k_bounding_sphere, dim3(1), dim3(1024), 0, use_front_stream(c), (const swr_vertex*)m->d_verts, (uint32_t)m->n_verts, m->d_bounds);
    SWR_HIP(c, hipGetLastError());
    m->bounds_ready = true;
    return SWR_OK;
}

static bool band_rejects(const swr_context* c, const swr_mesh* m, const float* model, const float* view, const float* proj) {
    if (!m->has_box || c->il_k > 0 || (c->band_ty0 <= 0 && c->band_ty1 >= c->tiles_y)) return false;
    double mv[16], M[16], amv[16], A[16];
    for (int r = 0; r < 4; ++r)
        for (int k = 0; k < 4; ++k) {
            double a = 0, b = 0;
            for (int j = 0; j < 4; ++j) { a += (double)model[r * 4 + j] * (double)view[j * 4 + k]; b += std::fabs((double)model[r * 4 + j]) * std::fabs((double)view[j * 4 + k]); }
            mv[r * 4 + k] = a; amv[r * 4 + k] = b;
        }
    for (int r = 0; r < 4; ++r)
        for (int k = 0; k < 4; ++k) {
            double a = 0, b = 0;
            for (int j = 0; j < 4; ++j) { a += mv[r * 4 + j] * (double)proj[j * 4 + k]; b += amv[r * 4 + j] * std::fabs((double)proj[j * 4 + k]); }
            M[r * 4 + k] = a; A[r * 4 + k] = b;
        }
    const double u16 = 16.0 / 16777216.0;
    double smin = 1e300, smax = -1e300, ey = 0, ew = 0, wmin = 1e300, ndc_abs = 0;
    for (int corner = 0; corner < 8; ++corner) {
        const double x = (corner & 1) ? m->box_hi[0] : m->box_lo[0];
        const double y = (corner & 2) ? m->box_hi[1] : m->box_lo[1];
        const double z = (corner & 4) ? m->box_hi[2] : m->box_lo[2];
        const double cy = x * M[1] + y * M[5] + z * M[9] + M[13];
        const double cw = x * M[3] + y * M[7] + z * M[11] + M[15];
        const double sy_abs = std::fabs(x) * A[1] + std::fabs(y) * A[5] + std::fabs(z) * A[9] + A[13];
        const double sw_abs = std::fabs(x) * A[3] + std::fabs(y) * A[7] + std::fabs(z) * A[11] + A[15];
        if (!std::isfinite(cy) || !std::isfinite(cw) || !std::isfinite(sy_abs) || !std::isfinite(sw_abs)) return false;
        ey = std::max(ey, u16 * sy_abs); ew = std::max(ew, u16 * sw_abs);
        if (!(cw > 0)) return false;
        wmin = std::min(wmin, cw);
        const double ndc = cy / cw;
        ndc_abs = std::max(ndc_abs, std::fabs(ndc));
        const double sy = (1.0 - (ndc * 0.5 + 0.5)) * (double)c->H;
        if (!std::isfinite(sy)) return false;
        smin = std::min(smin, sy); smax = std::max(smax, sy);
    }
    if (!(wmin - ew > 1e-6 * wmin)) return false;
    const double margin = 2.0 + 0.5 * (double)c->H * (ey + ndc_abs * ew) / (wmin - ew);
    if (!std::isfinite(margin)) return false;
    const double y0 = (double)band_y0(c), y1 = (double)std::min(c->H, c->band_ty1 * SWR_TILE);
    return smax + margin < y0 || smin - margin > y1;
}

int record_draw(swr_context* c, swr_mesh* mesh, const float* model, const float* view, const float* proj,
                int program, const swr_uniforms* u, const swr_texture* tex, int cull, int depth_test, int blend, bool frustum_cull = false) {
    if (!mesh || !model || !view || !proj) return fail(c, SWR_ERR_INVALID_ARG, "null argument to render_mesh");
    std::shared_ptr<UserProg> uprog;
    if (program >= SWR_PROG_USER_BASE) {
        auto it = c->progs.find(program);
        if (it == c->progs.end()) return fail(c, SWR_ERR_INVALID_ARG, "unknown or destroyed user program id");
        if (c->debug_mode == SWR_DEBUG_WIREFRAME)
            return fail(c, SWR_ERR_UNSUPPORTED, "user programs are not available in DebugMode.Wireframe");
        uprog = it->second;
    } else if (program < SWR_PROG_FLAT_COLOR || program > SWR_PROG_DEBUG_VARYINGS) {
        return fail(c, SWR_ERR_INVALID_ARG, "unknown program id");
    }
    if ((program == SWR_PROG_DUST2_LAMBERT_FOG || program == SWR_PROG_PHONG_4POINT) && !u)
        return fail(c, SWR_ERR_INVALID_ARG, "this program needs a uniform block");
    if (cull < 0 || cull > 2 || depth_test < 0 || depth_test > 7 || blend < 0 || blend > 3)
        return fail(c, SWR_ERR_INVALID_ARG, "enum value out of range");
    if (c->W <= 0 || c->H <= 0) return SWR_OK;
    const int n_tris = mesh->n_idx / 3;
    if (n_tris == 0) return SWR_OK;
    if (!(uprog && uprog->vertex_fn) && band_rejects(c, mesh, model, view, proj)) return SWR_OK;
    if ((uint64_t)mesh->n_verts + 4 * (uint64_t)n_tris >= (1ull << 26))
        return fail(c, SWR_ERR_UNSUPPORTED, "mesh exceeds 2^26 vertex-stage records (vertices + 4 x triangles: about 16.7 M triangles): split it");
    if (c->pend_verts + (uint64_t)mesh->n_verts + 4 * (c->pend_tris + (uint64_t)n_tris) >= (1ull << 26)) {
        int rc = flush_locked(c); if (rc) return rc;
    }
    if (!c->draws.empty() && kernel_class(c->draws.back().p.program) != kernel_class(program)) {
        int rc = flush_locked(c); if (rc) return rc;
    }
    DrawCmd d;
    memset(&d.p, 0, sizeof d.p);
    memcpy(d.p.model, model, 64); memcpy(d.p.view, view, 64); memcpy(d.p.proj, proj, 64);
    if (u) d.p.u = *u;
    d.p.verts = mesh->d_verts; d.p.idx = mesh->d_idx;
    d.p.tex = tex ? tex->d_rgba : nullptr;
    d.p.tex_w = tex ? tex->w : 0; d.p.tex_h = tex ? (tex->bilinear ? -tex->h : tex->h) : 0;
    if (tex && tex->bilinear && tex->d_blocked) { d.p.tex = tex->d_blocked; d.p.tex_w = -tex->w; }
    d.p.tex_wf = tex ? (float)tex->w : 0.0f; d.p.tex_hf = tex ? (float)tex->h : 0.0f;
    d.p.program = program; d.p.cull = cull; d.p.depth_test = depth_test; d.p.blend = blend;
    d.p.n_verts = (uint32_t)mesh->n_verts; d.p.n_tris = (uint32_t)n_tris;
    d.p.nm_flags = c->nm_flags;
    d.mesh = mesh;
    d.frustum_cull = frustum_cull;
    if (uprog) {
        d.uconsts = std::make_shared<const std::vector<float>>(uprog->constants, uprog->constants + 64);
        d.prog = std::move(uprog);
    }
    if (frustum_cull) { int rc = ensure_bounds(c, mesh); if (rc) return rc; }
    c->draws.push_back(d);
    c->pend_verts += mesh->n_verts; c->pend_tris += n_tris;
    return SWR_OK;
}

int make_mesh(swr_context* c, const swr_vertex* v, int nv, const uint16_t* idx, int ni, bool transient, swr_mesh** out) {
    if (nv < 0 || ni < 0 || (nv > 0 && !v) || (ni > 0 && !idx) || !out) return fail(c, SWR_ERR_INVALID_ARG, "bad mesh arguments");
    const int used = (ni / 3) * 3;
    for (int i = 0; i < used; ++i)
        if ((int)idx[i] >= nv) return fail(c, SWR_ERR_INVALID_ARG, "index out of range (C#: IndexOutOfRangeException)");
    swr_mesh* m = nullptr;
    if (transient) {
        size_t best = (size_t)-1;
        for (size_t i = 0; i < c->mesh_pool.size(); ++i) {
            swr_mesh* q = c->mesh_pool[i];
            if (q->cap_verts >= (size_t)nv * sizeof(swr_vertex) && q->cap_idx >= (size_t)ni * 2 + 8 &&
                (best == (size_t)-1 || q->cap_verts + q->cap_idx < c->mesh_pool[best]->cap_verts + c->mesh_pool[best]->cap_idx)) best = i;
        }
        if (best != (size_t)-1) {
            m = c->mesh_pool[best];
            c->mesh_pool.erase(c->mesh_pool.begin() + (std::ptrdiff_t)best);
            c->mesh_pool_bytes -= m->cap_verts + m->cap_idx;
            m->bounds_ready = false; m->has_box = false;
        }
    }
    if (!m) m = new swr_mesh();
    m->n_verts = nv; m->n_idx = ni; m->transient = transient;
    if (nv > 0) {
        bool ok = true;
        for (int k = 0; k < 3; ++k) { m->box_lo[k] = v[0].position[k]; m->box_hi[k] = v[0].position[k]; }
        for (int i = 0; i < nv; ++i)
            for (int k = 0; k < 3; ++k) {
                const float p = v[i].position[k];
                if (!(p == p)) ok = false;
                m->box_lo[k] = std::min(m->box_lo[k], p); m->box_hi[k] = std::max(m->box_hi[k], p);
            }
        m->has_box = ok;
    }
    hipError_t e = hipSuccess;
    if (nv && m->cap_verts < (size_t)nv * sizeof(swr_vertex)) {
        e = hipMalloc((void**)&m->d_verts, (size_t)nv * sizeof(swr_vertex));
        if (e == hipSuccess) m->cap_verts = (size_t)nv * sizeof(swr_vertex);
    }
    if (e == hipSuccess && ni && m->cap_idx < (size_t)ni * 2 + 8) {
        e = hipMalloc((void**)&m->d_idx, (size_t)ni * 2 + 8);
        if (e == hipSuccess) m->cap_idx = (size_t)ni * 2 + 8;
    }
    if (e == hipSuccess && nv) e = hipMemcpyAsync(m->d_verts, v, (size_t)nv * sizeof(swr_vertex), hipMemcpyHostToDevice, use_front_stream(c));
    if (e == hipSuccess && ni) e = hipMemcpyAsync(m->d_idx, idx, (size_t)ni * 2, hipMemcpyHostToDevice, use_front_stream(c));
    if (e != hipSuccess) {
        destroy_mesh(m);
        c->err = std::string("mesh upload failed: ") + hipGetErrorString(e);
        return e == hipErrorOutOfMemory ? SWR_ERR_OOM : SWR_ERR_HIP;
    }
    *out = m;
    return SWR_OK;
}

int present_is_stale(swr_context* c, int slot, bool& stale) {
    stale = false;
    if (!*(volatile uint32_t*)c->host_poison) return SWR_OK;
    Ctrl h;
    SWR_HIP(c, hipMemcpy(&h, c->d_ctrl.p, sizeof h, hipMemcpyDeviceToHost));
    stale = h.first_bad <= c->present_seq[slot];
    return SWR_OK;
}
}
```

### softwarerenderer_amd/csrc/swr_geometry.hip.h

```cpp
#pragma once
#include "swr_device.h"

namespace swr {

struct BlockMap { uint32_t draw; uint32_t first; };

#ifndef SWR_USER_VERTEX
__global__ __launch_bounds__(SWR_GEOM_BLOCK) void k_vertex(const DrawParams* __restrict__ draws,
                                                const BlockMap* __restrict__ blocks,
                                                VOut* __restrict__ vout, const uint32_t* __restrict__ visible,
                                                float* __restrict__ fog_r1_of_draw0 ,
                                                float4* __restrict__ vnorm ,
                                                uint32_t* __restrict__ zero_words, uint32_t n_zero ,
                                                uint32_t* __restrict__ zero_hist ) {
    SWR_FRONT_ENTER();
    for (uint32_t i = blockIdx.x * (uint32_t)SWR_GEOM_BLOCK + threadIdx.x; i < n_zero; i += gridDim.x * (uint32_t)SWR_GEOM_BLOCK) zero_words[i] = 0u;
    if (blockIdx.x == 0) for (uint32_t i = threadIdx.x; i < 512u; i += (uint32_t)SWR_GEOM_BLOCK) zero_hist[i] = 0u;
    const BlockMap bm = blocks[blockIdx.x];
    if (visible && !visible[bm.draw]) return;
    const DrawParams* __restrict__ dp = draws + bm.draw;
    const uint32_t local = bm.first + threadIdx.x;
    __shared__ float4 s_out[SWR_GEOM_BLOCK / 64][256];
    static_assert(sizeof(s_out) <= SWR_FRONT_MAX_LDS, "k_vertex must fit beside the raster kernel (swr_device.h)");
    float4 o0 = make_float4(0.f, 0.f, 0.f, 0.f), o1 = o0, o2 = o0, o3 = o0;
    const bool live = local < dp->n_verts;
    const uint32_t wv_ = threadIdx.x >> 6, lane_ = threadIdx.x & 63u;
    const uint32_t first_ = bm.first + wv_ * 64u;
    const uint32_t n_live_ = dp->n_verts > first_ ? min(dp->n_verts - first_, 64u) : 0u;
    {
        const float4* __restrict__ src = reinterpret_cast<const float4*>(dp->verts + first_);
        float4* sw = &s_out[wv_][0];
#pragma unroll
        for (int k = 0; k < 3; ++k) {
            const uint32_t e = (uint32_t)k * 64u + lane_;
            if (e < 3u * n_live_) sw[e] = src[e];
        }
        __builtin_amdgcn_fence(__ATOMIC_ACQ_REL, "workgroup");
        __builtin_amdgcn_wave_barrier();
    }
    if (live) {
    if (local == 0u) {
        const float den = dp->u.fog_end - dp->u.fog_start;
        fog_r1_of_draw0[(size_t)bm.draw * (sizeof(DrawParams) / sizeof(float))] = div_operand_safe(den) ? rcp_refined(den) : 0.0f;
        fog_r1_of_draw0[(size_t)bm.draw * (sizeof(DrawParams) / sizeof(float)) + 3] = den;
    }

    const float4 q0 = s_out[wv_][3 * lane_], q1 = s_out[wv_][3 * lane_ + 1], q2 = s_out[wv_][3 * lane_ + 2];

    float p[4] = { q0.x, q0.y, q0.z, 1.0f };
    float world[4], viewp[4], clip[4];
    const bool fma_t = (dp->nm_flags & SWR_NM_TRANSFORM_FMA) != 0u, fma_tn = (dp->nm_flags & SWR_NM_TRANSFORM_NORMAL_FMA) != 0u;
    vec4_transform(p, dp->model, world, fma_t);
    vec4_transform(world, dp->view, viewp, fma_t);
    vec4_transform(viewp, dp->proj, clip, fma_t);
    float n[3] = { q1.y, q1.z, q1.w }, tn[3];
    vec3_transform_normal(n, dp->model, tn, fma_tn);
    float len = sqrtf(dot3(tn[0], tn[1], tn[2], tn[0], tn[1], tn[2]));

    o0 = make_float4(clip[0], clip[1], clip[2], clip[3]);
    o1 = q2;
    o2 = make_float4(q0.w, q1.x, tn[0] / len, tn[1] / len);
    o3 = make_float4(tn[2] / len, world[0], world[1], world[2]);
    if (vnorm) vnorm[dp->vert_base + local] = make_float4(n[0], n[1], n[2], 0.0f);
    }
    {
        const uint32_t wv = wv_, lane = lane_;
        float4* sw = &s_out[wv][0];
        __builtin_amdgcn_fence(__ATOMIC_ACQ_REL, "workgroup");
        __builtin_amdgcn_wave_barrier();
        sw[4 * lane + 0] = o0; sw[4 * lane + 1] = o1; sw[4 * lane + 2] = o2; sw[4 * lane + 3] = o3;
        __builtin_amdgcn_fence(__ATOMIC_ACQ_REL, "workgroup");
        __builtin_amdgcn_wave_barrier();
        const uint32_t first = first_, n_live = n_live_;
        float4* dst = reinterpret_cast<float4*>(vout + dp->vert_base + first);
#pragma unroll
        for (int k = 0; k < 4; ++k) {
            const uint32_t e = (uint32_t)k * 64u + lane;
            if ((e >> 2) < n_live) dst[e] = sw[e];
        }
    }
}
#else
__global__ __launch_bounds__(SWR_GEOM_BLOCK) void k_vertex_user(const DrawParams* __restrict__ draws,
                                                const BlockMap* __restrict__ blocks,
                                                VOut* __restrict__ vout, const uint32_t* __restrict__ visible,
                                                float* __restrict__ fog_r1_of_draw0,
                                                float4* __restrict__ vnorm ,
                                                uint32_t* __restrict__ zero_words, uint32_t n_zero,
                                                uint32_t* __restrict__ zero_hist,
                                                const float* __restrict__ user_consts ) {
    SWR_FRONT_ENTER();
    for (uint32_t i = blockIdx.x * (uint32_t)SWR_GEOM_BLOCK + threadIdx.x; i < n_zero; i += gridDim.x * (uint32_t)SWR_GEOM_BLOCK) zero_words[i] = 0u;
    if (blockIdx.x == 0) for (uint32_t i = threadIdx.x; i < 512u; i += (uint32_t)SWR_GEOM_BLOCK) zero_hist[i] = 0u;
    const BlockMap bm = blocks[blockIdx.x];
    if (visible && !visible[bm.draw]) return;
    const DrawParams* __restrict__ dp = draws + bm.draw;
    const uint32_t local = bm.first + threadIdx.x;
    __shared__ float4 s_out[SWR_GEOM_BLOCK / 64][256];
    static_assert(sizeof(s_out) <= SWR_FRONT_MAX_LDS, "k_vertex_user must fit beside the raster kernel (swr_device.h)");
    float4 o0 = make_float4(0.f, 0.f, 0.f, 0.f), o1 = o0, o2 = o0, o3 = o0;
    const bool live = local < dp->n_verts;
    const uint32_t wv = threadIdx.x >> 6, lane = threadIdx.x & 63u;
    const uint32_t first = bm.first + wv * 64u;
    const uint32_t n_live = dp->n_verts > first ? min(dp->n_verts - first, 64u) : 0u;
    float4* sw = &s_out[wv][0];
    {
        const float4* __restrict__ src = reinterpret_cast<const float4*>(dp->verts + first);
#pragma unroll
        for (int k = 0; k < 3; ++k) {
            const uint32_t e = (uint32_t)k * 64u + lane;
            if (e < 3u * n_live) sw[e] = src[e];
        }
        __builtin_amdgcn_fence(__ATOMIC_ACQ_REL, "workgroup");
        __builtin_amdgcn_wave_barrier();
    }
    if (live) {
        if (local == 0u) {
            const float den = dp->u.fog_end - dp->u.fog_start;
            fog_r1_of_draw0[(size_t)bm.draw * (sizeof(DrawParams) / sizeof(float))] = div_operand_safe(den) ? rcp_refined(den) : 0.0f;
            fog_r1_of_draw0[(size_t)bm.draw * (sizeof(DrawParams) / sizeof(float)) + 3] = den;
        }
        const float4 q0 = sw[3 * lane], q1 = sw[3 * lane + 1], q2 = sw[3 * lane + 2];
        swr_vs_in in;
        in.position = make_float3(q0.x, q0.y, q0.z);
        in.uv = make_float2(q0.w, q1.x);
        in.normal = make_float3(q1.y, q1.z, q1.w);
        in.color = q2;
        const swr_vs_env env = { dp->model, dp->view, dp->proj, dp->u, user_consts + 64u * bm.draw, dp->nm_flags };
        swr_vs_out out;
        out.clip_position = make_float4(0.f, 0.f, 0.f, 0.f); out.color = make_float4(0.f, 0.f, 0.f, 0.f);
        out.tex_coord = make_float2(0.f, 0.f); out.normal = make_float3(0.f, 0.f, 0.f);
        out.world_normal = make_float3(0.f, 0.f, 0.f); out.data4 = make_float4(0.f, 0.f, 0.f, 0.f);
        swr_vertex(in, env, out);
        o0 = out.clip_position;
        o1 = out.color;
        o2 = make_float4(out.tex_coord.x, out.tex_coord.y, out.world_normal.x, out.world_normal.y);
        o3 = make_float4(out.world_normal.z, out.data4.x, out.data4.y, out.data4.z);
        vnorm[dp->vert_base + local] = make_float4(out.normal.x, out.normal.y, out.normal.z, out.data4.w);
    }
    {
        __builtin_amdgcn_fence(__ATOMIC_ACQ_REL, "workgroup");
        __builtin_amdgcn_wave_barrier();
        sw[4 * lane + 0] = o0; sw[4 * lane + 1] = o1; sw[4 * lane + 2] = o2; sw[4 * lane + 3] = o3;
        __builtin_amdgcn_fence(__ATOMIC_ACQ_REL, "workgroup");
        __builtin_amdgcn_wave_barrier();
        float4* dst = reinterpret_cast<float4*>(vout + dp->vert_base + first);
#pragma unroll
        for (int k = 0; k < 4; ++k) {
            const uint32_t e = (uint32_t)k * 64u + lane;
            if ((e >> 2) < n_live) dst[e] = sw[e];
        }
    }
}
#endif

struct SVert {
    VOut v; bool interp; float nrm[3];
#ifdef SWR_USER_VERTEX
    float d4w;
#endif
};

__device__ __forceinline__ void svert_lerp(const SVert& a, const SVert& b, float t, SVert& r) {
#pragma unroll
    for (int i = 0; i < 4; ++i) r.v.clip[i] = nm_lerp(a.v.clip[i], b.v.clip[i], t);
#pragma unroll
    for (int i = 0; i < 2; ++i) r.v.uv[i] = nm_lerp(a.v.uv[i], b.v.uv[i], t);
#pragma unroll
    for (int i = 0; i < 4; ++i) r.v.color[i] = nm_lerp(a.v.color[i], b.v.color[i], t);
#pragma unroll
    for (int i = 0; i < 3; ++i) r.v.wn[i] = nm_lerp(a.v.wn[i], b.v.wn[i], t);
#pragma unroll
    for (int i = 0; i < 3; ++i) r.v.wpos[i] = nm_lerp(a.v.wpos[i], b.v.wpos[i], t);
#pragma unroll
    for (int i = 0; i < 3; ++i) r.nrm[i] = nm_lerp(a.nrm[i], b.nrm[i], t);
#ifdef SWR_USER_VERTEX
    r.d4w = nm_lerp(a.d4w, b.d4w, t);
#endif
    r.interp = true;
}

__device__ __forceinline__ void store_vout(VOut* __restrict__ dst, const VOut& v) {
    float4* o = reinterpret_cast<float4*>(dst);
    o[0] = make_float4(v.clip[0], v.clip[1], v.clip[2], v.clip[3]);
    o[1] = make_float4(v.color[0], v.color[1], v.color[2], v.color[3]);
    o[2] = make_float4(v.uv[0], v.uv[1], v.wn[0], v.wn[1]);
    o[3] = make_float4(v.wn[2], v.wpos[0], v.wpos[1], v.wpos[2]);
}
__device__ __forceinline__ void load_vout(const VOut* __restrict__ src, VOut& v) {
    const float4* s = reinterpret_cast<const float4*>(src);
    float4 a = s[0], b = s[1], c = s[2], d = s[3];
    v.clip[0] = a.x; v.clip[1] = a.y; v.clip[2] = a.z; v.clip[3] = a.w;
    v.color[0] = b.x; v.color[1] = b.y; v.color[2] = b.z; v.color[3] = b.w;
    v.uv[0] = c.x; v.uv[1] = c.y; v.wn[0] = c.z; v.wn[1] = c.w;
    v.wn[2] = d.x; v.wpos[0] = d.y; v.wpos[1] = d.z; v.wpos[2] = d.w;
}

__device__ __forceinline__ int setup_triangle(const FrameParams& fp, int cull, uint32_t draw,
                                              const SVert& v0, const SVert& v1, const SVert& v2,
                                              uint32_t r0, uint32_t r1, uint32_t r2,
                                              TriRec* __restrict__ rec, unsigned long long* __restrict__ tb, uint32_t* __restrict__ wnt,
                                              bool wireframe,
                                              float4* __restrict__ rec_regs = nullptr ) {
    const int rw = fp.width, rh = fp.height;
    const SVert* o[3] = { &v2, &v1, &v0 };
    float sx[3], sy[3], dz[3];
#pragma unroll
    for (int i = 0; i < 3; ++i) {
        float invW = 1.0f / o[i]->v.clip[3];
        float nx = o[i]->v.clip[0] * invW, ny = o[i]->v.clip[1] * invW, nz = o[i]->v.clip[2] * invW;
        if (is_nan_or_inf(nx) || is_nan_or_inf(ny) || is_nan_or_inf(nz)) return 0;
        sx[i] = (nx * 0.5f + 0.5f) * (float)rw;
        sy[i] = (1.0f - (ny * 0.5f + 0.5f)) * (float)rh;
        dz[i] = (nz + 1.0f) * 0.5f;
    }
    if (v0.v.clip[3] == 0 || v1.v.clip[3] == 0 || v2.v.clip[3] == 0) return 0;
    float area = edge_function(sx[0], sy[0], sx[1], sy[1], sx[2], sy[2]);
    if (area == 0) return 0;
    bool front = area < 0;
    if ((cull == SWR_CULL_BACK && !front) || (cull == SWR_CULL_FRONT && front)) return 0;
    const uint32_t flags = draw | (o[0]->interp ? SWR_FLAG_INTERP : 0u);

    if (wireframe) {
#pragma unroll
        for (int e = 0; e < 3; ++e) {
            const int i0 = e, i1 = (e + 1) % 3;
            const float p0x = sx[i0], p0y = sy[i0], p1x = sx[i1], p1y = sy[i1];
            const int minX = f2i(mathf_max(mathf_min(p0x, p1x), 0.0f));
            const int maxX = f2i(mathf_min(mathf_max(p0x, p1x), (float)(rw - 1)));
            const int minY = f2i(mathf_max(mathf_min(p0y, p1y), 0.0f));
            const int maxY = f2i(mathf_min(mathf_max(p0y, p1y), (float)(rh - 1)));
            if (minX > maxX || minY > maxY) continue;
            float4* out = reinterpret_cast<float4*>(rec + e);
            out[0] = make_float4(p0x, p1x, 0.0f, p0y);
            out[1] = make_float4(p1y, 0.0f, dz[0], dz[1]);
            out[2] = make_float4(dz[2], 0.0f, __uint_as_float(r2), __uint_as_float(r1));
            out[3] = make_float4(__uint_as_float(r2),
                                 __uint_as_float((uint32_t)minX | ((uint32_t)maxX << 16)),
                                 __uint_as_float((uint32_t)minY | ((uint32_t)maxY << 16)),
                                 __uint_as_float(flags | SWR_FLAG_LINE));
            tb[e] = (unsigned long long)(minX / SWR_TILE) | ((unsigned long long)(maxX / SWR_TILE) << 16) |
                    ((unsigned long long)(minY / SWR_TILE) << 32) | ((unsigned long long)(maxY / SWR_TILE) << 48);
            wnt[e] = small_want_mask(band_map(fp), tb[e], sx, sy, minX, maxX, minY, maxY, rw, rh, true);
        }
        return 0;
    }

    float inv_area = 1.0f / area;
    float minXf = mathf_min(mathf_min(sx[0], sx[1]), sx[2]);
    float maxXf = mathf_max(mathf_max(sx[0], sx[1]), sx[2]);
    float minYf = mathf_min(mathf_min(sy[0], sy[1]), sy[2]);
    float maxYf = mathf_max(mathf_max(sy[0], sy[1]), sy[2]);
    int minX = max(f2i(floorf(minXf)), 0);
    int maxX = min(f2i(ceilf(maxXf)), rw - 1);
    int minY = max(f2i(floorf(minYf)), 0);
    int maxY = min(f2i(ceilf(maxYf)), rh - 1);
    if (minX > maxX || minY > maxY) return 0;

    float4* out = rec_regs ? rec_regs : reinterpret_cast<float4*>(rec);
    {
    out[0] = make_float4(sx[0], sx[1], sx[2], sy[0]);
    out[1] = make_float4(sy[1], sy[2], dz[0], dz[1]);
    out[2] = make_float4(dz[2], inv_area, __uint_as_float(r2), __uint_as_float(r1));
    out[3] = make_float4(__uint_as_float(r0),
                         __uint_as_float((uint32_t)minX | ((uint32_t)maxX << 16)),
                         __uint_as_float((uint32_t)minY | ((uint32_t)maxY << 16)),
                         __uint_as_float(flags));
    }
    tb[0] = (unsigned long long)(minX / SWR_TILE) | ((unsigned long long)(maxX / SWR_TILE) << 16) |
            ((unsigned long long)(minY / SWR_TILE) << 32) | ((unsigned long long)(maxY / SWR_TILE) << 48);
    wnt[0] = small_want_mask(band_map(fp), tb[0], sx, sy, minX, maxX, minY, maxY, rw, rh, false);
    return 1;
}

#define SWR_FRAG_DRAW(dp, bm) ((dp)->frag_draw)
__global__ __launch_bounds__(SWR_GEOM_BLOCK) void k_setup(const DrawParams* __restrict__ draws,
                                               const BlockMap* __restrict__ blocks,
                                               const VOut* __restrict__ vout_ro,
                                               VOut* __restrict__ clip_pool,
                                               uint32_t clip_pool_base,
                                               TriRec* __restrict__ recs,
                                               uint32_t odd_base,
                                               unsigned long long* __restrict__ slot_tb,
                                               uint8_t* __restrict__ want,
                                               FrameParams fp,
                                               Counters* __restrict__ counters ,
                                               const Ctrl* __restrict__ ctrl, uint32_t seq, int count_stats, int wireframe,
                                               const uint32_t* __restrict__ visible,
                                               float4* __restrict__ vnorm ) {
    SWR_FRONT_ENTER();
    const BlockMap bm = blocks[blockIdx.x];
    const DrawParams* __restrict__ dp = draws + bm.draw;
    const uint32_t local = bm.first + threadIdx.x;
    const bool in_range = local < dp->n_tris;
    const bool drawn = !visible || visible[bm.draw] != 0u;
    const bool active = in_range && drawn;
    unsigned n_setup = 0, n_clipped = 0;
    float4 rec_q[4] = { make_float4(0.f, 0.f, 0.f, 0.f), make_float4(0.f, 0.f, 0.f, 0.f), make_float4(0.f, 0.f, 0.f, 0.f), make_float4(0.f, 0.f, 0.f, 0.f) };
    bool rec_valid = false;

    if (in_range && !drawn) {
        const uint32_t per_fan = wireframe ? 3u : 1u;
        const uint32_t slot = 2u * per_fan * (dp->tri_base + local);
        for (uint32_t k = 0; k < 2u * per_fan; ++k) slot_tb[slot + k] = SWR_TB_INVALID;
    }
    if (active) {
        const uint32_t gt = dp->tri_base + local;
        const uint32_t per_fan = wireframe ? 3u : 1u;
        const uint32_t slot = 2u * per_fan * gt;
        unsigned long long tbs[6] = { SWR_TB_INVALID, SWR_TB_INVALID, SWR_TB_INVALID, SWR_TB_INVALID, SWR_TB_INVALID, SWR_TB_INVALID };
        uint32_t wnt[6] = { 0u, 0u, 0u, 0u, 0u, 0u };

        const uint16_t* __restrict__ ip = dp->idx + 3u * local;
        const uint32_t r0 = dp->vert_base + ip[0], r1 = dp->vert_base + ip[1], r2 = dp->vert_base + ip[2];
        SVert v[3];
        {
            const float4 c0 = reinterpret_cast<const float4*>(vout_ro + r0)[0], c1 = reinterpret_cast<const float4*>(vout_ro + r1)[0],
                         c2 = reinterpret_cast<const float4*>(vout_ro + r2)[0];
            v[0].v.clip[0] = c0.x; v[0].v.clip[1] = c0.y; v[0].v.clip[2] = c0.z; v[0].v.clip[3] = c0.w;
            v[1].v.clip[0] = c1.x; v[1].v.clip[1] = c1.y; v[1].v.clip[2] = c1.z; v[1].v.clip[3] = c1.w;
            v[2].v.clip[0] = c2.x; v[2].v.clip[1] = c2.y; v[2].v.clip[2] = c2.z; v[2].v.clip[3] = c2.w;
        }
        const bool interp = dp->program != SWR_PROG_FLAT_COLOR;
        v[0].interp = v[1].interp = v[2].interp = interp;

        const bool b0 = v[0].v.clip[3] <= 0, b1 = v[1].v.clip[3] <= 0, b2 = v[2].v.clip[3] <= 0;
        if (!(b0 && b1 && b2)) {
            if (b0 || b1 || b2) {
                n_clipped = 1;
                load_vout(vout_ro + r0, v[0].v);
                load_vout(vout_ro + r1, v[1].v);
                load_vout(vout_ro + r2, v[2].v);
                if (vnorm) {
                    const float4 n0 = vnorm[r0], n1 = vnorm[r1], n2 = vnorm[r2];
                    v[0].nrm[0] = n0.x; v[0].nrm[1] = n0.y; v[0].nrm[2] = n0.z;
                    v[1].nrm[0] = n1.x; v[1].nrm[1] = n1.y; v[1].nrm[2] = n1.z;
                    v[2].nrm[0] = n2.x; v[2].nrm[1] = n2.y; v[2].nrm[2] = n2.z;
#ifdef SWR_USER_VERTEX
                    v[0].d4w = n0.w; v[1].d4w = n1.w; v[2].d4w = n2.w;
#endif
                } else {
                    for (int i = 0; i < 3; ++i) v[i].nrm[0] = v[i].nrm[1] = v[i].nrm[2] = 0.0f;
#ifdef SWR_USER_VERTEX
                    for (int i = 0; i < 3; ++i) v[i].d4w = 0.0f;
#endif
                }
                SVert poly[4];
                int n = 0;
                const float nearc = fp.near_clip;
#pragma unroll
                for (int i = 0; i < 3; ++i) {
                    const SVert& cur = v[i];
                    const SVert& nxt = v[(i + 1) % 3];
                    bool cur_in = cur.v.clip[2] >= nearc * cur.v.clip[3];
                    bool nxt_in = nxt.v.clip[2] >= nearc * nxt.v.clip[3];
                    if (cur_in) { poly[n & 3] = cur; ++n; }
                    if (cur_in != nxt_in) {
                        float z0 = cur.v.clip[2], w0 = cur.v.clip[3], z1 = nxt.v.clip[2], w1 = nxt.v.clip[3];
                        float denom = (z1 - z0) - nearc * (w1 - w0);
                        float t;
                        if (fabsf(denom) < SWR_EPSILON) {
                            t = 0.5f;
                        } else {
                            t = (z0 - nearc * w0) / (nearc * (w1 - w0) - (z1 - z0));
                            t = math_clamp(t, 0.0f, 1.0f);
                        }
                        svert_lerp(cur, nxt, t, poly[n & 3]); ++n;
                    }
                }
                if (n >= 3) {
                    VOut* pool = clip_pool + 4ull * gt;
                    const uint32_t pbase = clip_pool_base + 4u * gt;
                    for (int k = 0; k < n; ++k) store_vout(pool + k, poly[k].v);
#ifdef SWR_USER_VERTEX
                    if (vnorm) for (int k = 0; k < n; ++k) vnorm[pbase + (uint32_t)k] = make_float4(poly[k].nrm[0], poly[k].nrm[1], poly[k].nrm[2], poly[k].d4w);
#else
                    if (vnorm) for (int k = 0; k < n; ++k) vnorm[pbase + (uint32_t)k] = make_float4(poly[k].nrm[0], poly[k].nrm[1], poly[k].nrm[2], 0.0f);
#endif
                    n_setup += setup_triangle(fp, dp->cull, SWR_FRAG_DRAW(dp, bm), poly[0], poly[1], poly[2],
                                              pbase, pbase + 1, pbase + 2, recs + rec_index(slot, odd_base), &tbs[0], &wnt[0], wireframe != 0);
                    if (n == 4) n_setup += setup_triangle(fp, dp->cull, SWR_FRAG_DRAW(dp, bm), poly[0], poly[2], poly[3],
                                                          pbase, pbase + 2, pbase + 3, recs + rec_index(slot + per_fan, odd_base), &tbs[3], &wnt[3], wireframe != 0);
                }
            } else {
                if (!wireframe) {
                    rec_valid = setup_triangle(fp, dp->cull, SWR_FRAG_DRAW(dp, bm), v[0], v[1], v[2], r0, r1, r2, nullptr, &tbs[0], &wnt[0], false, rec_q) != 0;
                    n_setup += rec_valid ? 1u : 0u;
                } else
                n_setup += setup_triangle(fp, dp->cull, SWR_FRAG_DRAW(dp, bm), v[0], v[1], v[2], r0, r1, r2, recs + rec_index(slot, odd_base), &tbs[0], &wnt[0], wireframe != 0);
            }
        }
        if (wireframe) {
#pragma unroll
            for (int k = 0; k < 6; ++k) { slot_tb[slot + k] = tbs[k]; want[slot + k] = (uint8_t)wnt[k]; }
        } else {
            *reinterpret_cast<ulonglong2*>(slot_tb + slot) = make_ulonglong2(tbs[0], tbs[3]);
            *reinterpret_cast<uint16_t*>(want + slot) = (uint16_t)(wnt[0] | (wnt[3] << 8));
        }
    }

    {
        __shared__ float4 s_rec[SWR_GEOM_BLOCK / 64][256];
        static_assert(sizeof(s_rec) + 16 <= SWR_FRONT_MAX_LDS, "k_setup must fit beside the raster kernel (swr_device.h)");
        const uint32_t wv = threadIdx.x >> 6, lane = threadIdx.x & 63u;
        const unsigned long long vmask = __ballot(rec_valid);
        if (vmask) {
            float4* sw = &s_rec[wv][0];
            sw[4 * lane + 0] = rec_q[0]; sw[4 * lane + 1] = rec_q[1]; sw[4 * lane + 2] = rec_q[2]; sw[4 * lane + 3] = rec_q[3];
            __builtin_amdgcn_fence(__ATOMIC_ACQ_REL, "workgroup");
            __builtin_amdgcn_wave_barrier();
            const uint32_t slot0 = 2u * (dp->tri_base + bm.first + wv * 64u);
            float4* dst = reinterpret_cast<float4*>(recs);
#pragma unroll
            for (int k = 0; k < 4; ++k) {
                const uint32_t e = (uint32_t)k * 64u + lane, j = e >> 2;
                if ((vmask >> j) & 1ull) dst[4u * (size_t)rec_index(slot0 + 2u * j, odd_base) + (e & 3u)] = sw[e];
            }
        }
    }
    __shared__ unsigned s_cnt[3];
    if (threadIdx.x < 3) s_cnt[threadIdx.x] = 0;
    __syncthreads();
    unsigned long long act_mask = __ballot(active);
    unsigned long long set_mask1 = __ballot(n_setup >= 1), set_mask2 = __ballot(n_setup >= 2);
    unsigned long long clip_mask = __ballot(n_clipped != 0);
    if ((threadIdx.x & 63) == 0) {
        atomicAdd(&s_cnt[0], (unsigned)__popcll(act_mask));
        atomicAdd(&s_cnt[1], (unsigned)(__popcll(set_mask1) + __popcll(set_mask2)));
        atomicAdd(&s_cnt[2], (unsigned)__popcll(clip_mask));
    }
    __syncthreads();
    if (threadIdx.x == 0 && count_stats && !batch_poisoned(ctrl, seq)) {
        Counters* c = counters + (blockIdx.x & 63);
        atomicAdd(&c->triangles_in, (unsigned long long)s_cnt[0]);
        if (s_cnt[1]) atomicAdd(&c->triangles_setup, (unsigned long long)s_cnt[1]);
        if (s_cnt[2]) atomicAdd(&c->triangles_clipped, (unsigned long long)s_cnt[2]);
    }
}

}
```

### softwarerenderer_amd/csrc/swr_host.h

```cpp
#pragma once

struct swr_mesh {
    float4* d_bounds = nullptr;
    bool bounds_ready = false;
    swr_vertex* d_verts = nullptr;
    uint16_t* d_idx = nullptr;
    int n_verts = 0, n_idx = 0;
    size_t cap_verts = 0, cap_idx = 0;
    bool transient = false;
    float box_lo[3] = { 0, 0, 0 }, box_hi[3] = { 0, 0, 0 };
    bool has_box = false;
};
struct swr_texture {
    uint8_t* d_rgba = nullptr;
    uint8_t* d_blocked = nullptr;
    int w = 0, h = 0;
    bool bilinear = false;
};

namespace {

thread_local std::string g_create_error;

struct DevBuf {
    void* p = nullptr;
    size_t cap = 0;
    template <class T> T* as() const { return reinterpret_cast<T*>(p); }
};

enum Stage { ST_VERTEX = 0, ST_SETUP, ST_BIN, ST_SORT, ST_COVER, ST_RASTER, ST_CLEAR, ST_COUNT };

struct EventSpan { int stage; hipEvent_t a, b; };

#ifndef SWR_TIMING_EVENT_FLAGS
#define SWR_TIMING_EVENT_FLAGS hipEventDisableSystemFence
#endif
#ifndef SWR_HANDOVER_EVENT_FLAGS
#define SWR_HANDOVER_EVENT_FLAGS hipEventDisableTiming
#endif
#define SWR_SLOTS 3
struct FrameSlot { void* host = nullptr; size_t cap = 0; hipEvent_t done = nullptr; bool busy = false; };

struct RasterSet {
    DevBuf d_upload;
    DevBuf d_vout, d_vnorm, d_recs;
    DevBuf d_masks, d_pcounts, d_pair_refs;
    DevBuf d_tile_count, d_tile_start;
    DevBuf d_order;
    uint32_t hist_tiles = 0;
    hipEvent_t front_done = nullptr, raster_done = nullptr;
    bool raster_pending = false;
};

struct UserProg {
    hipModule_t mod = nullptr;
    hipFunction_t fn[2] = { nullptr, nullptr };
    hipFunction_t vertex_fn = nullptr, setup_fn = nullptr;
    float constants[64] = {};
    ~UserProg() { if (mod) (void)hipModuleUnload(mod); }
};

struct DrawCmd {
    DrawParams p;
    swr_mesh* mesh;
    bool frustum_cull = false;
    std::shared_ptr<UserProg> prog;
    std::shared_ptr<const std::vector<float>> uconsts;
};

struct Batch {
    std::vector<DrawCmd> draws;
    bool clear_color = false, clear_depth = false;
    float clear_rgba[4] = { 0, 0, 0, 0 };
    float near_clip = 0.1f;
    bool wireframe = false;
    uint32_t seq = 0;
    float4* color = nullptr;
    float* depth = nullptr;
};

}

struct swr_context {
    int device = 0;
    std::mutex mu;
    std::string err;
    hipStream_t own_stream = nullptr, stream = nullptr;
    hipStream_t front_stream = nullptr;
    int pipelining = 1;
    uint32_t pipeline_max_tris = 1u << 17;
    uint32_t pipeline_max_tiles = 1u << 15;
    hipEvent_t f_tail_ev = nullptr, r_front_ev = nullptr;
    bool f_tail_pending = false;
    bool r_front_pending = false;
    RasterSet sets[2];
    uint32_t raster_span_no = 0;
    char dev_name[256] = { 0 };

    int W = 0, H = 0, tiles_x = 0, tiles_y = 0;
    bool geometry_applied = false;
    bool band_set = false;
    int band_first = 0, band_count = 0;
    int band_ty0 = 0, band_ty1 = 0;
    int il_k = 0, il_world = 1, il_rank = 0;
    int band_tile_rows = 0;
    float4* color = nullptr;
    float* depth = nullptr;
    DevBuf own_color, own_depth;
    void* ext_color = nullptr; void* ext_depth = nullptr;

    uint32_t nm_flags = SWR_NUMERICS_FMA ? (SWR_NM_TRANSFORM_FMA | SWR_NM_TRANSFORM_NORMAL_FMA) : 0u;
    float near_clip = 0.1f, far_clip = 1000.0f;
    int debug_mode = SWR_DEBUG_NONE;

    bool pend_clear_color = false, pend_clear_depth = false;
    float clear_rgba[4] = { 0, 0, 0, 0 };

    std::vector<DrawCmd> draws;
    uint64_t pend_verts = 0, pend_tris = 0;
    std::vector<swr_mesh*> garbage;
    std::map<int, std::shared_ptr<UserProg>> progs;
    int next_prog = SWR_PROG_USER_BASE;
    std::vector<std::shared_ptr<UserProg>> prog_garbage;
    std::vector<swr_mesh*> mesh_pool;
    size_t mesh_pool_bytes = 0;
    uint64_t stale_dropped[2] = { 0, 0 };
    std::vector<Batch> inflight;
    uint32_t next_seq = 1;
    bool sync_flush = false;
    uint32_t debug_fill_capacity = 0;

    DevBuf d_slot_tb;
    FrameSlot slots[SWR_SLOTS];
    uint32_t slot_next = 0;
    DevBuf d_pair_tile, d_ctrl;
    uint32_t* host_poison = nullptr;
    DevBuf d_tile_list, d_tile_stats, d_counters, d_total, d_scratch;
    DevBuf d_want;
    size_t tile_stats_tiles = 0;
    swr_stats totals = {};
    unsigned long long host_tile_pairs = 0;
    unsigned long long replays = 0;
    unsigned long long host_syncs = 0;
    hipStream_t copy_stream = nullptr;
    DevBuf present_buf[2];
    hipEvent_t present_flat[2] = { nullptr, nullptr }, present_done[2] = { nullptr, nullptr };
    uint64_t present_ticket[2] = { 0, 0 };
    uint32_t present_seq[2] = { 0, 0 };
    uint64_t next_ticket = 0;

    int profiling = 0;
    std::vector<EventSpan> spans;
    std::vector<float> raster_samples;
    std::vector<hipEvent_t> event_pool;
    swr_profile prof = {};
};

namespace {

#define SWR_HIP(ctx, call)                                                                        \
    do {                                                                                          \
        hipError_t e_ = (call);                                                                   \
        if (e_ != hipSuccess) {                                                                   \
            char b_[512];                                                                         \
            snprintf(b_, sizeof b_, "%s failed: %s (%s:%d)", #call, hipGetErrorString(e_), __FILE__, __LINE__); \
            (ctx)->err = b_;                                                                      \
            return e_ == hipErrorOutOfMemory ? SWR_ERR_OOM : SWR_ERR_HIP;                         \
        }                                                                                         \
    } while (0)

int fail(swr_context* c, int code, const char* msg) { c->err = msg; return code; }

int ensure(swr_context* c, DevBuf& b, size_t bytes, bool zero_new = false) {
    if (bytes <= b.cap) return SWR_OK;
    size_t want = std::max(bytes, b.cap + b.cap / 2);
    if (b.p) { SWR_HIP(c, hipFree(b.p)); b.p = nullptr; b.cap = 0; }
    SWR_HIP(c, hipMalloc(&b.p, want));
    b.cap = want;
    if (zero_new) SWR_HIP(c, hipMemsetAsync(b.p, 0, want, c->stream));
    return SWR_OK;
}

void release(DevBuf& b) { if (b.p) (void)hipFree(b.p); b.p = nullptr; b.cap = 0; }

void* slot_acquire(swr_context* c, size_t bytes) {
    FrameSlot& fs = c->slots[c->slot_next % SWR_SLOTS];
    if (fs.busy) { (void)hipEventSynchronize(fs.done); fs.busy = false; }
    if (fs.cap < bytes) {
        if (fs.host) (void)hipHostFree(fs.host);
        fs.host = nullptr; fs.cap = 0;
        size_t cap = std::max<size_t>(bytes + bytes / 2, 1 << 16);
        if (hipHostMalloc(&fs.host, cap, hipHostMallocDefault) != hipSuccess) { fs.host = nullptr; return nullptr; }
        fs.cap = cap;
    }
    return fs.host;
}
void slot_submit(swr_context* c) {
    FrameSlot& fs = c->slots[c->slot_next % SWR_SLOTS];
    if (!fs.done) (void)hipEventCreateWithFlags(&fs.done, hipEventDisableTiming);
    if (fs.done && hipEventRecord(fs.done, c->stream) == hipSuccess) fs.busy = true;
    c->slot_next++;
}

BandMap host_band_map(const swr_context* c) {
    BandMap b; b.ty0 = c->band_ty0; b.ty1 = c->band_ty1; b.il_k = c->il_k; b.il_world = c->il_world; b.il_rank = c->il_rank;
    return b;
}
int band_y0(const swr_context* c) { return c->band_ty0 * SWR_TILE; }
int band_rows(const swr_context* c) {
    if (c->band_tile_rows <= 0) return 0;
    const int last_global = band_global_row(host_band_map(c), c->band_tile_rows - 1);
    const int last_rows = std::min(SWR_TILE, c->H - last_global * SWR_TILE);
    return (c->band_tile_rows - 1) * SWR_TILE + std::max(0, last_rows);
}
int band_local_pixel_row(const swr_context* c, int y) {
    if (y < 0 || y >= c->H) return -1;
    const int lr = band_local_row(host_band_map(c), y / SWR_TILE);
    return lr < 0 ? -1 : lr * SWR_TILE + y % SWR_TILE;
}
size_t band_pixels(const swr_context* c) { return (size_t)std::max(0, c->W) * (size_t)band_rows(c); }

int apply_geometry(swr_context* c) {
    c->tiles_x = c->W > 0 ? (c->W + SWR_TILE - 1) / SWR_TILE : 0;
    c->tiles_y = c->H > 0 ? (c->H + SWR_TILE - 1) / SWR_TILE : 0;
    if (c->il_k > 0) {
        c->band_ty0 = 0; c->band_ty1 = c->tiles_y;
        int rows = 0;
        for (int ty = 0; ty < c->tiles_y; ++ty) rows += band_local_row(host_band_map(c), ty) >= 0 ? 1 : 0;
        c->band_tile_rows = rows;
    } else {
        if (c->band_set) {
            c->band_ty0 = std::min(std::max(c->band_first, 0), c->tiles_y);
            c->band_ty1 = std::min(c->band_ty0 + std::max(c->band_count, 0), c->tiles_y);
        } else {
            c->band_ty0 = 0; c->band_ty1 = c->tiles_y;
        }
        c->band_tile_rows = c->band_ty1 - c->band_ty0;
    }
    size_t n = band_pixels(c);
    if (c->ext_color) {
        c->color = (float4*)c->ext_color; c->depth = (float*)c->ext_depth;
    } else {
        int rc;
        if ((rc = ensure(c, c->own_color, std::max<size_t>(n, 1) * sizeof(float4), false))) return rc;
        if ((rc = ensure(c, c->own_depth, std::max<size_t>(n, 1) * sizeof(float), false))) return rc;
        c->color = c->own_color.as<float4>(); c->depth = c->own_depth.as<float>();
    }
    return SWR_OK;
}

FrameParams frame_params(const swr_context* c, float near_clip) {
    FrameParams fp;
    fp.width = c->W; fp.height = c->H; fp.tiles_x = c->tiles_x; fp.tiles_y = c->tiles_y;
    fp.band_ty0 = c->band_ty0; fp.band_ty1 = c->band_ty1;
    fp.band_y0 = band_y0(c); fp.band_rows = band_rows(c);
    fp.il_k = c->il_k; fp.il_world = c->il_world; fp.il_rank = c->il_rank; fp.band_tile_rows = c->band_tile_rows;
    fp.near_clip = near_clip;
    return fp;
}

hipEvent_t get_event(swr_context* c) {
    if (!c->event_pool.empty()) { hipEvent_t e = c->event_pool.back(); c->event_pool.pop_back(); return e; }
    hipEvent_t e = nullptr;
    if (hipEventCreateWithFlags(&e, SWR_TIMING_EVENT_FLAGS) != hipSuccess) (void)hipEventCreate(&e);
    return e;
}
struct ScopedSpan {
    swr_context* c; int stage; hipEvent_t a = nullptr, b = nullptr;
    hipStream_t s;
    bool on = false;
    ScopedSpan(swr_context* c_, int st, hipStream_t s_ = nullptr) : c(c_), stage(st), s(s_ ? s_ : c_->stream) {
        on = c->profiling == 1 || (st == ST_RASTER && (c->profiling == 2 || (c->profiling == 3 && (c->raster_span_no++ & 3u) == 0u)));
        if (on) { a = get_event(c); b = get_event(c); (void)hipEventRecord(a, s); }
    }
    ~ScopedSpan() {
        if (on) { (void)hipEventRecord(b, s); c->spans.push_back({ stage, a, b }); }
    }
};

void collect_spans(swr_context* c) {
    for (auto& s : c->spans) {
        float ms = 0.f;
        if (hipEventElapsedTime(&ms, s.a, s.b) == hipSuccess) {
            switch (s.stage) {
            case ST_VERTEX: c->prof.vertex_ms += ms; break;
            case ST_SETUP:  c->prof.setup_ms += ms; break;
            case ST_BIN:    c->prof.bin_ms += ms; break;
            case ST_SORT:   c->prof.sort_ms += ms; break;
            case ST_COVER:  c->prof.cover_ms += ms; break;
            case ST_RASTER: c->prof.raster_ms += ms; c->prof.raster_launches++;
                            if (c->raster_samples.size() < 65536) c->raster_samples.push_back(ms);
                            break;
            case ST_CLEAR:  c->prof.clear_ms += ms; break;
            }
            c->prof.total_ms += ms;
        }
        c->event_pool.push_back(s.a); c->event_pool.push_back(s.b);
    }
    c->spans.clear();
}

hipStream_t use_front_stream(swr_context* c) {
    if (c->pipelining && c->front_stream) { c->f_tail_pending = true; return c->front_stream; }
    return c->stream;
}

int ensure_front_stream(swr_context* c) {
    if (!c->pipelining || c->front_stream) return SWR_OK;
    int least = 0, greatest = 0;
    SWR_HIP(c, hipDeviceGetStreamPriorityRange(&least, &greatest));
    SWR_HIP(c, hipStreamCreateWithPriority(&c->front_stream, hipStreamNonBlocking, greatest));
    SWR_HIP(c, hipEventCreateWithFlags(&c->f_tail_ev, hipEventDisableTiming));
    SWR_HIP(c, hipEventCreateWithFlags(&c->r_front_ev, hipEventDisableTiming));
    for (auto& s : c->sets) {
        if (!s.front_done) SWR_HIP(c, hipEventCreateWithFlags(&s.front_done, SWR_HANDOVER_EVENT_FLAGS));
        if (!s.raster_done) SWR_HIP(c, hipEventCreateWithFlags(&s.raster_done, SWR_HANDOVER_EVENT_FLAGS));
    }
    return SWR_OK;
}
}
```

Before: 78410 Mfragments/s.

## Fuse tile-count binning pass into the triangle setup kernel

```diff
diff --git a/softwarerenderer_amd/csrc/swr_api.hip b/softwarerenderer_amd/csrc/swr_api.hip
--- a/softwarerenderer_amd/csrc/swr_api.hip
+++ b/softwarerenderer_amd/csrc/swr_api.hip
@@ -138,6 +138,7 @@
     { const char* sf = getenv("SWR_SYNC_FLUSH"); c->sync_flush = sf && sf[0] == '1'; }
 #ifdef SWR_TEST_HOOKS
     { const char* df = getenv("SWR_DEBUG_FILL_CAPACITY"); c->debug_fill_capacity = df ? (uint32_t)strtoul(df, nullptr, 10) : 0u; }
+    { const char* dm = getenv("SWR_DEBUG_MAX_PAIRS"); c->debug_max_pairs = dm ? strtoull(dm, nullptr, 10) : 0ull; }
 #endif
     int rc = ensure(c, c->d_counters, 65 * sizeof(Counters));
     if (!rc) rc = ensure(c, c->d_ctrl, 64);
diff --git a/softwarerenderer_amd/csrc/swr_bin_combine.hip.h b/softwarerenderer_amd/csrc/swr_bin_combine.hip.h
--- /dev/null
+++ b/softwarerenderer_amd/csrc/swr_bin_combine.hip.h
@@ -0,0 +1,209 @@
+#pragma once
+#include "swr_device.h"
+
+namespace swr {
+
+struct BinArgs {
+    const unsigned long long* __restrict__ slot_tb;
+    const TriRec* __restrict__ recs;
+    uint32_t odd_base;
+    uint32_t slot_lo, slot_hi;
+    uint32_t spt;
+    int tiles_x;
+    BandMap band;
+    int width, height;
+    uint32_t* __restrict__ tile_count;
+    const uint32_t* __restrict__ tile_start;
+    uint32_t* __restrict__ tile_list;
+    uint32_t list_capacity;
+    Counters* __restrict__ counters;
+    Ctrl* __restrict__ ctrl;
+    uint32_t seq;
+    uint32_t replayable;
+    const unsigned long long* __restrict__ total;
+    const uint8_t* __restrict__ want;
+    uint32_t tpw;
+    uint32_t bin_blocks;
+    int order_tiles_y;
+    const uint8_t* __restrict__ tile_bucket;
+    const uint32_t* __restrict__ order_hist;
+    uint32_t* __restrict__ order_cursor;
+    uint4* __restrict__ tile_order;
+};
+
+__device__ __forceinline__ void bin_overflow(const BinArgs& a) {
+    a.counters->overflow = 1u;
+    if (a.ctrl->host_flag) __hip_atomic_store(a.ctrl->host_flag + 1, 1u, __ATOMIC_RELAXED, __HIP_MEMORY_SCOPE_SYSTEM);
+    if (a.replayable) {
+        atomicMin(&a.ctrl->first_bad, a.seq);
+        atomicMax(&a.ctrl->need, 2ull * (unsigned long long)a.list_capacity + 4096ull);
+        __hip_atomic_store(&a.ctrl->poison, 1u, __ATOMIC_RELAXED, __HIP_MEMORY_SCOPE_AGENT);
+        if (a.ctrl->host_flag) __hip_atomic_store(a.ctrl->host_flag, 1u, __ATOMIC_RELAXED, __HIP_MEMORY_SCOPE_SYSTEM);
+    }
+}
+
+struct SlotData {
+    int tminx, tminy, nx, ny;
+    float sx[3], sy[3];
+    int minX, maxX, minY, maxY;
+    bool is_line;
+};
+__device__ __forceinline__ SlotData slot_data(const BandMap& band, unsigned long long tb, const float4& r0, const float4& r1, const float4& r3) {
+    SlotData s;
+    s.sx[0] = s.sx[1] = s.sx[2] = s.sy[0] = s.sy[1] = s.sy[2] = 0.f;
+    s.minX = s.minY = 0; s.maxX = s.maxY = -1; s.is_line = false;
+    SlotTiles st;
+    slot_tiles(band, tb, st);
+    s.tminx = st.tminx; s.tminy = st.tminy; s.nx = st.nx; s.ny = st.ny;
+    if (s.nx * s.ny > SWR_SMALL_TILES) {
+        s.sx[0] = r0.x; s.sx[1] = r0.y; s.sx[2] = r0.z; s.sy[0] = r0.w; s.sy[1] = r1.x; s.sy[2] = r1.y;
+        const uint32_t bbx = __float_as_uint(r3.y), bby = __float_as_uint(r3.z);
+        s.minX = (int)(bbx & 0xffffu); s.maxX = (int)(bbx >> 16); s.minY = (int)(bby & 0xffffu); s.maxY = (int)(bby >> 16);
+        s.is_line = (__float_as_uint(r3.w) & SWR_FLAG_LINE) != 0u;
+    }
+    return s;
+}
+
+template <bool FILL>
+__device__ __forceinline__ void bin_big(const BinArgs& a, const SlotData& sd, uint32_t slot, bool big) {
+    const int lane = threadIdx.x & 63;
+    const int nt = sd.nx * sd.ny;
+    unsigned long long med = __ballot(big && nt <= 64);
+    while (med) {
+        bool want[4];
+        uint32_t tile[4], sslot[4], base[4];
+#pragma unroll
+        for (int j = 0; j < 4; ++j) {
+            want[j] = false; tile[j] = 0u; sslot[j] = 0u; base[j] = 0u;
+            if (med) {
+                const int src = __ffsll((long long)med) - 1;
+                med &= med - 1;
+                const int s_tminx = __shfl(sd.tminx, src), s_tminy = __shfl(sd.tminy, src);
+                const int s_nx = __shfl(sd.nx, src), s_nt = __shfl(nt, src);
+                sslot[j] = (uint32_t)__shfl((int)slot, src);
+                float bsx[3], bsy[3];
+#pragma unroll
+                for (int k = 0; k < 3; ++k) { bsx[k] = __shfl(sd.sx[k], src); bsy[k] = __shfl(sd.sy[k], src); }
+                const int bminX = __shfl(sd.minX, src), bmaxX = __shfl(sd.maxX, src), bminY = __shfl(sd.minY, src), bmaxY = __shfl(sd.maxY, src);
+                const bool b_line = __shfl((int)sd.is_line, src) != 0;
+                if (lane < s_nt) {
+                    const int ty = s_tminy + lane / s_nx, tx = s_tminx + lane % s_nx;
+                    want[j] = band_local_row(a.band, ty) >= 0 && pair_may_cover(bsx, bsy, bminX, bmaxX, bminY, bmaxY, tx, ty, a.width, a.height, b_line);
+                    tile[j] = (uint32_t)(band_local_row(a.band, ty) * a.tiles_x + tx);
+                }
+                if (want[j]) {
+                    if (FILL) base[j] = atomicAdd(&a.tile_count[tile[j]], 1u);
+                    else atomicAdd(&a.tile_count[tile[j]], 1u);
+                }
+            }
+        }
+        if (FILL) {
+#pragma unroll
+            for (int j = 0; j < 4; ++j) {
+                if (want[j]) {
+                    const uint32_t at = a.tile_start[tile[j]] + base[j];
+                    if (at < a.list_capacity) a.tile_list[at] = sslot[j];
+                    else bin_overflow(a);
+                }
+            }
+        }
+    }
+    unsigned long long m = __ballot(big && nt > 64);
+    while (m) {
+        const int src = __ffsll((long long)m) - 1;
+        m &= m - 1;
+        const int s_tminx = __shfl(sd.tminx, src), s_tminy = __shfl(sd.tminy, src);
+        const int s_nx = __shfl(sd.nx, src), s_nt = __shfl(nt, src);
+        const uint32_t s_slot = (uint32_t)__shfl((int)slot, src);
+        float bsx[3], bsy[3];
+#pragma unroll
+        for (int k = 0; k < 3; ++k) { bsx[k] = __shfl(sd.sx[k], src); bsy[k] = __shfl(sd.sy[k], src); }
+        const int bminX = __shfl(sd.minX, src), bmaxX = __shfl(sd.maxX, src), bminY = __shfl(sd.minY, src), bmaxY = __shfl(sd.maxY, src);
+        const bool b_line = __shfl((int)sd.is_line, src) != 0;
+        for (int i0 = 0; i0 < s_nt; i0 += 64) {
+            const int i = i0 + lane;
+            bool want = i < s_nt;
+            int ty = 0, tx = 0;
+            if (want) {
+                ty = s_tminy + i / s_nx; tx = s_tminx + i % s_nx;
+                want = band_local_row(a.band, ty) >= 0 && pair_may_cover(bsx, bsy, bminX, bmaxX, bminY, bmaxY, tx, ty, a.width, a.height, b_line);
+            }
+            if (want) {
+                const uint32_t tile = (uint32_t)(band_local_row(a.band, ty) * a.tiles_x + tx);
+                if (FILL) {
+                    const uint32_t at = a.tile_start[tile] + atomicAdd(&a.tile_count[tile], 1u);
+                    if (at < a.list_capacity) a.tile_list[at] = s_slot;
+                    else bin_overflow(a);
+                } else {
+                    atomicAdd(&a.tile_count[tile], 1u);
+                }
+            }
+        }
+    }
+}
+
+#define SWR_BIN_TABLE_LOG2 8
+#define SWR_BIN_TABLE (1 << SWR_BIN_TABLE_LOG2)
+template <bool FILL, int THREADS>
+__device__ __forceinline__ void bin_block_slots(const BinArgs& a, const SlotData& sd, uint32_t slot, uint32_t want_in, uint32_t* s_key, uint32_t* s_val) {
+    const int nt = sd.nx * sd.ny;
+    const bool big = nt > SWR_SMALL_TILES;
+    const int nt_small = big ? 0 : nt;
+    if (!__syncthreads_or(nt != 0)) return;
+    for (int e = threadIdx.x; e < SWR_BIN_TABLE; e += THREADS) { s_key[e] = 0u; s_val[e] = 0u; }
+    __syncthreads();
+    uint32_t packed[SWR_SMALL_TILES];
+    SlotTiles st; st.tminx = sd.tminx; st.tminy = sd.tminy; st.nx = sd.nx; st.ny = sd.ny;
+    SmallTileWalk w(st);
+    const uint32_t wmask = nt_small ? want_in : 0u;
+#pragma unroll
+    for (int i = 0; i < SWR_SMALL_TILES; ++i) {
+        packed[i] = 0u;
+        if (i < nt_small) {
+            if ((wmask >> i) & 1u) {
+                const uint32_t tile = (uint32_t)(band_local_row(a.band, w.ty) * a.tiles_x + w.tx);
+                uint32_t e = (tile * 0x9E3779B1u) >> (32 - SWR_BIN_TABLE_LOG2);
+                bool placed = false;
+                for (int probe = 0; probe < 16; ++probe) {
+                    const uint32_t prev = atomicCAS(&s_key[e], 0u, tile + 1u);
+                    if (prev == 0u || prev == tile + 1u) { placed = true; break; }
+                    e = (e + 1u) & (SWR_BIN_TABLE - 1u);
+                }
+                if (placed) {
+                    const uint32_t rank = atomicAdd(&s_val[e], 1u);
+                    packed[i] = e | (rank << 12) | 0x80000000u;
+                } else if (FILL) {
+                    const uint32_t at = a.tile_start[tile] + atomicAdd(&a.tile_count[tile], 1u);
+                    if (at < a.list_capacity) a.tile_list[at] = slot;
+                    else bin_overflow(a);
+                } else {
+                    atomicAdd(&a.tile_count[tile], 1u);
+                }
+            }
+            w.next();
+        }
+    }
+    __syncthreads();
+    for (int e = threadIdx.x; e < SWR_BIN_TABLE; e += THREADS) {
+        const uint32_t key = s_key[e];
+        if (key) {
+            const uint32_t tile = key - 1u, n = s_val[e];
+            if (FILL) s_val[e] = a.tile_start[tile] + atomicAdd(&a.tile_count[tile], n);
+            else atomicAdd(&a.tile_count[tile], n);
+        }
+    }
+    if (FILL) {
+        __syncthreads();
+#pragma unroll
+        for (int i = 0; i < SWR_SMALL_TILES; ++i) {
+            if (packed[i] & 0x80000000u) {
+                const uint32_t at = s_val[packed[i] & 0xfffu] + ((packed[i] >> 12) & 0x7ffffu);
+                if (at < a.list_capacity) a.tile_list[at] = slot;
+                else bin_overflow(a);
+            }
+        }
+    }
+    bin_big<FILL>(a, sd, slot, big);
+}
+
+}
diff --git a/softwarerenderer_amd/csrc/swr_binning.hip.h b/softwarerenderer_amd/csrc/swr_binning.hip.h
--- a/softwarerenderer_amd/csrc/swr_binning.hip.h
+++ b/softwarerenderer_amd/csrc/swr_binning.hip.h
@@ -1,49 +1,11 @@
 #pragma once
 #include "swr_device.h"
+#include "swr_bin_combine.hip.h"
 
 #define SWR_ORDER_BUCKETS 256
 
 namespace swr {
 
-struct BinArgs {
-    const unsigned long long* __restrict__ slot_tb;
-    const TriRec* __restrict__ recs;
-    uint32_t odd_base;
-    uint32_t slot_lo, slot_hi;
-    uint32_t spt;
-    int tiles_x;
-    BandMap band;
-    int width, height;
-    uint32_t* __restrict__ tile_count;
-    const uint32_t* __restrict__ tile_start;
-    uint32_t* __restrict__ tile_list;
-    uint32_t list_capacity;
-    Counters* __restrict__ counters;
-    Ctrl* __restrict__ ctrl;
-    uint32_t seq;
-    uint32_t replayable;
-    const unsigned long long* __restrict__ total;
-    const uint8_t* __restrict__ want;
-    uint32_t tpw;
-    uint32_t bin_blocks;
-    int order_tiles_y;
-    const uint8_t* __restrict__ tile_bucket;
-    const uint32_t* __restrict__ order_hist;
-    uint32_t* __restrict__ order_cursor;
-    uint4* __restrict__ tile_order;
-};
-
-
-__device__ __forceinline__ void bin_overflow(const BinArgs& a) {
-    a.counters->overflow = 1u;
-    if (a.ctrl->host_flag) __hip_atomic_store(a.ctrl->host_flag + 1, 1u, __ATOMIC_RELAXED, __HIP_MEMORY_SCOPE_SYSTEM);
-    if (a.replayable) {
-        atomicMin(&a.ctrl->first_bad, a.seq);
-        atomicMax(&a.ctrl->need, 2ull * (unsigned long long)a.list_capacity + 4096ull);
-        __hip_atomic_store(&a.ctrl->poison, 1u, __ATOMIC_RELAXED, __HIP_MEMORY_SCOPE_AGENT);
-        if (a.ctrl->host_flag) __hip_atomic_store(a.ctrl->host_flag, 1u, __ATOMIC_RELAXED, __HIP_MEMORY_SCOPE_SYSTEM);
-    }
-}
 
 __device__ __forceinline__ uint32_t order_bucket(uint32_t w) {
     if (w == 0u) return 0u;
@@ -92,171 +54,15 @@
     }
 }
 
-struct SlotData {
-    int tminx, tminy, nx, ny;
-    float sx[3], sy[3];
-    int minX, maxX, minY, maxY;
-    bool is_line;
-};
 __device__ __forceinline__ SlotData slot_load(const BinArgs& a, uint32_t slot, unsigned long long tb) {
-    SlotData s;
-    s.sx[0] = s.sx[1] = s.sx[2] = s.sy[0] = s.sy[1] = s.sy[2] = 0.f;
-    s.minX = s.minY = 0; s.maxX = s.maxY = -1; s.is_line = false;
     SlotTiles st;
     slot_tiles(a.band, tb, st);
-    s.tminx = st.tminx; s.tminy = st.tminy; s.nx = st.nx; s.ny = st.ny;
-    if (s.nx * s.ny > SWR_SMALL_TILES) {
+    float4 r0 = make_float4(0.f, 0.f, 0.f, 0.f), r1 = r0, r3 = r0;
+    if (st.nx * st.ny > SWR_SMALL_TILES) {
         const float4* __restrict__ rq = reinterpret_cast<const float4*>(a.recs + rec_index(slot, a.odd_base));
-        const float4 r0 = rq[0], r1 = rq[1], r3 = rq[3];
-        s.sx[0] = r0.x; s.sx[1] = r0.y; s.sx[2] = r0.z; s.sy[0] = r0.w; s.sy[1] = r1.x; s.sy[2] = r1.y;
-        const uint32_t bbx = __float_as_uint(r3.y), bby = __float_as_uint(r3.z);
-        s.minX = (int)(bbx & 0xffffu); s.maxX = (int)(bbx >> 16); s.minY = (int)(bby & 0xffffu); s.maxY = (int)(bby >> 16);
-        s.is_line = (__float_as_uint(r3.w) & SWR_FLAG_LINE) != 0u;
-    }
-    return s;
-}
-
-template <bool FILL>
-__device__ __forceinline__ void bin_big(const BinArgs& a, const SlotData& sd, uint32_t slot, bool big) {
-    const int lane = threadIdx.x & 63;
-    const int nt = sd.nx * sd.ny;
-    unsigned long long med = __ballot(big && nt <= 64);
-    while (med) {
-        bool want[4];
-        uint32_t tile[4], sslot[4], base[4];
-#pragma unroll
-        for (int j = 0; j < 4; ++j) {
-            want[j] = false; tile[j] = 0u; sslot[j] = 0u; base[j] = 0u;
-            if (med) {
-                const int src = __ffsll((long long)med) - 1;
-                med &= med - 1;
-                const int s_tminx = __shfl(sd.tminx, src), s_tminy = __shfl(sd.tminy, src);
-                const int s_nx = __shfl(sd.nx, src), s_nt = __shfl(nt, src);
-                sslot[j] = (uint32_t)__shfl((int)slot, src);
-                float bsx[3], bsy[3];
-#pragma unroll
-                for (int k = 0; k < 3; ++k) { bsx[k] = __shfl(sd.sx[k], src); bsy[k] = __shfl(sd.sy[k], src); }
-                const int bminX = __shfl(sd.minX, src), bmaxX = __shfl(sd.maxX, src), bminY = __shfl(sd.minY, src), bmaxY = __shfl(sd.maxY, src);
-                const bool b_line = __shfl((int)sd.is_line, src) != 0;
-                if (lane < s_nt) {
-                    const int ty = s_tminy + lane / s_nx, tx = s_tminx + lane % s_nx;
-                    want[j] = band_local_row(a.band, ty) >= 0 && pair_may_cover(bsx, bsy, bminX, bmaxX, bminY, bmaxY, tx, ty, a.width, a.height, b_line);
-                    tile[j] = (uint32_t)(band_local_row(a.band, ty) * a.tiles_x + tx);
-                }
-                if (want[j]) {
-                    if (FILL) base[j] = atomicAdd(&a.tile_count[tile[j]], 1u);
-                    else atomicAdd(&a.tile_count[tile[j]], 1u);
-                }
-            }
-        }
-        if (FILL) {
-#pragma unroll
-            for (int j = 0; j < 4; ++j) {
-                if (want[j]) {
-                    const uint32_t at = a.tile_start[tile[j]] + base[j];
-                    if (at < a.list_capacity) a.tile_list[at] = sslot[j];
-                    else bin_overflow(a);
-                }
-            }
-        }
-    }
-    unsigned long long m = __ballot(big && nt > 64);
-    while (m) {
-        const int src = __ffsll((long long)m) - 1;
-        m &= m - 1;
-        const int s_tminx = __shfl(sd.tminx, src), s_tminy = __shfl(sd.tminy, src);
-        const int s_nx = __shfl(sd.nx, src), s_nt = __shfl(nt, src);
-        const uint32_t s_slot = (uint32_t)__shfl((int)slot, src);
-        float bsx[3], bsy[3];
-#pragma unroll
-        for (int k = 0; k < 3; ++k) { bsx[k] = __shfl(sd.sx[k], src); bsy[k] = __shfl(sd.sy[k], src); }
-        const int bminX = __shfl(sd.minX, src), bmaxX = __shfl(sd.maxX, src), bminY = __shfl(sd.minY, src), bmaxY = __shfl(sd.maxY, src);
-        const bool b_line = __shfl((int)sd.is_line, src) != 0;
-        for (int i0 = 0; i0 < s_nt; i0 += 64) {
-            const int i = i0 + lane;
-            bool want = i < s_nt;
-            int ty = 0, tx = 0;
-            if (want) {
-                ty = s_tminy + i / s_nx; tx = s_tminx + i % s_nx;
-                want = band_local_row(a.band, ty) >= 0 && pair_may_cover(bsx, bsy, bminX, bmaxX, bminY, bmaxY, tx, ty, a.width, a.height, b_line);
-            }
-            if (want) {
-                const uint32_t tile = (uint32_t)(band_local_row(a.band, ty) * a.tiles_x + tx);
-                if (FILL) {
-                    const uint32_t at = a.tile_start[tile] + atomicAdd(&a.tile_count[tile], 1u);
-                    if (at < a.list_capacity) a.tile_list[at] = s_slot;
-                    else bin_overflow(a);
-                } else {
-                    atomicAdd(&a.tile_count[tile], 1u);
-                }
-            }
-        }
-    }
-}
-
-#define SWR_BIN_TABLE_LOG2 8
-#define SWR_BIN_TABLE (1 << SWR_BIN_TABLE_LOG2)
-template <bool FILL>
-__device__ __forceinline__ void bin_block_slots(const BinArgs& a, uint32_t slot, unsigned long long tb, uint32_t want_in, uint32_t* s_key, uint32_t* s_val) {
-    const SlotData sd = slot_load(a, slot, tb);
-    const int nt = sd.nx * sd.ny;
-    const bool big = nt > SWR_SMALL_TILES;
-    const int nt_small = big ? 0 : nt;
-    if (!__syncthreads_or(nt != 0)) return;
-    for (int e = threadIdx.x; e < SWR_BIN_TABLE; e += 256) { s_key[e] = 0u; s_val[e] = 0u; }
-    __syncthreads();
-    uint32_t packed[SWR_SMALL_TILES];
-    SlotTiles st; st.tminx = sd.tminx; st.tminy = sd.tminy; st.nx = sd.nx; st.ny = sd.ny;
-    SmallTileWalk w(st);
-    const uint32_t wmask = nt_small ? want_in : 0u;
-#pragma unroll
-    for (int i = 0; i < SWR_SMALL_TILES; ++i) {
-        packed[i] = 0u;
-        if (i < nt_small) {
-            if ((wmask >> i) & 1u) {
-                const uint32_t tile = (uint32_t)(band_local_row(a.band, w.ty) * a.tiles_x + w.tx);
-                uint32_t e = (tile * 0x9E3779B1u) >> (32 - SWR_BIN_TABLE_LOG2);
-                bool placed = false;
-                for (int probe = 0; probe < 16; ++probe) {
-                    const uint32_t prev = atomicCAS(&s_key[e], 0u, tile + 1u);
-                    if (prev == 0u || prev == tile + 1u) { placed = true; break; }
-                    e = (e + 1u) & (SWR_BIN_TABLE - 1u);
-                }
-                if (placed) {
-                    const uint32_t rank = atomicAdd(&s_val[e], 1u);
-                    packed[i] = e | (rank << 12) | 0x80000000u;
-                } else if (FILL) {
-                    const uint32_t at = a.tile_start[tile] + atomicAdd(&a.tile_count[tile], 1u);
-                    if (at < a.list_capacity) a.tile_list[at] = slot;
-                    else bin_overflow(a);
-                } else {
-                    atomicAdd(&a.tile_count[tile], 1u);
-                }
-            }
-            w.next();
-        }
-    }
-    __syncthreads();
-    for (int e = threadIdx.x; e < SWR_BIN_TABLE; e += 256) {
-        const uint32_t key = s_key[e];
-        if (key) {
-            const uint32_t tile = key - 1u, n = s_val[e];
-            if (FILL) s_val[e] = a.tile_start[tile] + atomicAdd(&a.tile_count[tile], n);
-            else atomicAdd(&a.tile_count[tile], n);
-        }
-    }
-    if (FILL) {
-        __syncthreads();
-#pragma unroll
-        for (int i = 0; i < SWR_SMALL_TILES; ++i) {
-            if (packed[i] & 0x80000000u) {
-                const uint32_t at = s_val[packed[i] & 0xfffu] + ((packed[i] >> 12) & 0x7ffffu);
-                if (at < a.list_capacity) a.tile_list[at] = slot;
-                else bin_overflow(a);
-            }
-        }
-    }
-    bin_big<FILL>(a, sd, slot, big);
+        r0 = rq[0]; r1 = rq[1]; r3 = rq[3];
+    }
+    return slot_data(a.band, tb, r0, r1, r3);
 }
 
 template <bool FILL>
@@ -281,7 +87,7 @@
     for (uint32_t si = 0; si < a.spt; ++si) {
         const unsigned long long tb_next = tb_of(si + 1);
         const uint32_t wm_next = want_of(si + 1);
-        bin_block_slots<FILL>(a, first + si, tb, wm, s_key, s_val);
+        bin_block_slots<FILL, 256>(a, slot_load(a, first + si, tb), first + si, wm, s_key, s_val);
         tb = tb_next; wm = wm_next;
     }
 }
diff --git a/softwarerenderer_amd/csrc/swr_flush.h b/softwarerenderer_amd/csrc/swr_flush.h
--- a/softwarerenderer_amd/csrc/swr_flush.h
+++ b/softwarerenderer_amd/csrc/swr_flush.h
@@ -131,7 +131,7 @@
 
 int launch_raster(swr_context* c, Pass& P, uint32_t n_tiles);
 
-int bin_and_raster(swr_context* c, Pass& P, uint32_t lo, uint32_t hi, bool counts_clear = false) {
+int bin_and_raster(swr_context* c, Pass& P, uint32_t lo, uint32_t hi, bool counts_clear = false, bool counted = false) {
     const uint32_t n_tiles = (uint32_t)c->tiles_x * (uint32_t)c->band_tile_rows;
     if (n_tiles == 0 || lo >= hi) return SWR_OK;
     int rc;
@@ -168,7 +168,7 @@
             SWR_HIP(c, hipMemsetAsync(ba.tile_count, 0, (size_t)n_tiles * 4, F));
             SWR_HIP(c, hipMemsetAsync(ov.hist, 0, 2 * SWR_ORDER_BUCKETS * 4, F));
         }
-        hipLaunchKernelGGL(k_bin<false>, dim3(bin_blocks), dim3(256), 0, F, ba);
+        if (!counted) hipLaunchKernelGGL(k_bin<false>, dim3(bin_blocks), dim3(256), 0, F, ba);
         const unsigned scan_blocks = (n_tiles + (unsigned)SWR_SCAN_BLOCK - 1u) / (unsigned)SWR_SCAN_BLOCK;
         unsigned long long* sums = d_total + 32;
         hipLaunchKernelGGL(k_scan_sums, dim3(scan_blocks), dim3(SWR_SCAN_BLOCK), 0, F, (const uint32_t*)ba.tile_count, n_tiles, sums);
@@ -184,7 +184,7 @@
         unsigned long long total = 0;
         SWR_HIP(c, hipMemcpyAsync(&total, d_total, 8, hipMemcpyDeviceToHost, F));
         SWR_HIP(c, hipStreamSynchronize(F));
-        if (total > kMaxPairs && hi - lo > 2) {
+        if (total > (c->debug_max_pairs ? c->debug_max_pairs : kMaxPairs) && hi - lo > 2) {
             uint32_t mid = lo + (((hi - lo) / 2u) & ~1u);
             if (mid == lo) mid = lo + 2;
             if ((rc = bin_and_raster(c, P, lo, mid))) return rc;
@@ -337,7 +337,7 @@
     return g;
 }
 
-int launch_geometry(swr_context* c, const Pass& P, const BatchGeometry& g, uint32_t n_tiles, int count_stats) {
+int launch_geometry(swr_context* c, const Pass& P, const BatchGeometry& g, uint32_t n_tiles, int count_stats, bool setup_counts) {
     const Batch& b = P.b; RasterSet& S = P.S; const hipStream_t F = P.F;
     const UserProg* vprog = b_has_user_vertex(b) ? b.draws[0].prog.get() : nullptr;
     const auto launch = [&](hipFunction_t user_fn, const void* builtin, size_t blocks, void** args) {
@@ -383,8 +383,9 @@
         const Ctrl* a_ctrl = c->d_ctrl.as<Ctrl>();
         uint32_t a_seq = b.seq;
         int a_count = count_stats, a_wire = b.wireframe ? 1 : 0;
+        uint32_t* a_tile_count = setup_counts ? S.d_tile_count.as<uint32_t>() : (uint32_t*)nullptr;
         void* args[] = { &d_draws, &d_tblocks, &a_vout, &a_pool, &a_pool_base, &a_recs, &a_odd_base, &a_tb, &a_want, &fp, &a_counters, &a_ctrl, &a_seq,
-                         &a_count, &a_wire, &d_visible, &a_vnorm };
+                         &a_count, &a_wire, &d_visible, &a_vnorm, &a_tile_count };
         SWR_HIP(c, launch(vprog ? vprog->setup_fn : nullptr, (const void*)k_setup, g.tblocks.size(), args));
     }
     return SWR_OK;
@@ -463,9 +464,10 @@
         for (size_t i = 0; i < nd; ++i) memcpy(uc + 64 * i, b.draws[i].uconsts->data(), 64 * sizeof(float));
     }
     SWR_HIP(c, hipMemcpyAsync(S.d_upload.p, stage, P.up.bytes, hipMemcpyHostToDevice, F));
-    if ((rc = launch_geometry(c, P, g, n_tiles, count_stats))) return rc;
     const bool counts_clear = !g.vblocks.empty() && n_tiles != 0;
-    rc = bin_and_raster(c, P, 0, (uint32_t)(spt * T), counts_clear);
+    const bool setup_counts = counts_clear && !b.wireframe;
+    if ((rc = launch_geometry(c, P, g, n_tiles, count_stats, setup_counts))) return rc;
+    rc = bin_and_raster(c, P, 0, (uint32_t)(spt * T), counts_clear, setup_counts);
     slot_submit(c);
     if (rc) return rc;
     if (c->pipelining && mode != MODE_ASYNC) SWR_HIP(c, hipStreamSynchronize(c->stream));
diff --git a/softwarerenderer_amd/csrc/swr_geometry.hip.h b/softwarerenderer_amd/csrc/swr_geometry.hip.h
--- a/softwarerenderer_amd/csrc/swr_geometry.hip.h
+++ b/softwarerenderer_amd/csrc/swr_geometry.hip.h
@@ -1,5 +1,6 @@
 #pragma once
 #include "swr_device.h"
+#include "swr_bin_combine.hip.h"
 
 namespace swr {
 
@@ -287,7 +288,8 @@
                                                Counters* __restrict__ counters ,
                                                const Ctrl* __restrict__ ctrl, uint32_t seq, int count_stats, int wireframe,
                                                const uint32_t* __restrict__ visible,
-                                               float4* __restrict__ vnorm ) {
+                                               float4* __restrict__ vnorm ,
+                                               uint32_t* __restrict__ tile_count ) {
     SWR_FRONT_ENTER();
     const BlockMap bm = blocks[blockIdx.x];
     const DrawParams* __restrict__ dp = draws + bm.draw;
@@ -298,6 +300,9 @@
     unsigned n_setup = 0, n_clipped = 0;
     float4 rec_q[4] = { make_float4(0.f, 0.f, 0.f, 0.f), make_float4(0.f, 0.f, 0.f, 0.f), make_float4(0.f, 0.f, 0.f, 0.f), make_float4(0.f, 0.f, 0.f, 0.f) };
     bool rec_valid = false;
+    unsigned long long cnt_tb0 = SWR_TB_INVALID, cnt_tb1 = SWR_TB_INVALID;
+    uint32_t cnt_want = 0u;
+    float4 odd_q0 = make_float4(0.f, 0.f, 0.f, 0.f), odd_q1 = odd_q0, odd_q3 = odd_q0;
 
     if (in_range && !drawn) {
         const uint32_t per_fan = wireframe ? 3u : 1u;
@@ -377,10 +382,27 @@
 #else
                     if (vnorm) for (int k = 0; k < n; ++k) vnorm[pbase + (uint32_t)k] = make_float4(poly[k].nrm[0], poly[k].nrm[1], poly[k].nrm[2], 0.0f);
 #endif
-                    n_setup += setup_triangle(fp, dp->cull, SWR_FRAG_DRAW(dp, bm), poly[0], poly[1], poly[2],
-                                              pbase, pbase + 1, pbase + 2, recs + rec_index(slot, odd_base), &tbs[0], &wnt[0], wireframe != 0);
-                    if (n == 4) n_setup += setup_triangle(fp, dp->cull, SWR_FRAG_DRAW(dp, bm), poly[0], poly[2], poly[3],
-                                                          pbase, pbase + 2, pbase + 3, recs + rec_index(slot + per_fan, odd_base), &tbs[3], &wnt[3], wireframe != 0);
+                    float4 fan_e[4], fan_q[4];
+                    TriRec* const rec_e = recs + rec_index(slot, odd_base);
+                    const int ok_e = setup_triangle(fp, dp->cull, SWR_FRAG_DRAW(dp, bm), poly[0], poly[1], poly[2],
+                                                    pbase, pbase + 1, pbase + 2, rec_e, &tbs[0], &wnt[0], wireframe != 0, fan_e);
+                    n_setup += ok_e;
+                    if (ok_e && !wireframe) {
+                        float4* o = reinterpret_cast<float4*>(rec_e);
+                        o[0] = fan_e[0]; o[1] = fan_e[1]; o[2] = fan_e[2]; o[3] = fan_e[3];
+                        rec_q[0] = fan_e[0]; rec_q[1].x = fan_e[1].x; rec_q[1].y = fan_e[1].y; rec_q[3] = fan_e[3];
+                    }
+                    if (n == 4) {
+                        TriRec* const rec_o = recs + rec_index(slot + per_fan, odd_base);
+                        const int ok_o = setup_triangle(fp, dp->cull, SWR_FRAG_DRAW(dp, bm), poly[0], poly[2], poly[3],
+                                                        pbase, pbase + 2, pbase + 3, rec_o, &tbs[3], &wnt[3], wireframe != 0, fan_q);
+                        n_setup += ok_o;
+                        if (ok_o && !wireframe) {
+                            float4* o = reinterpret_cast<float4*>(rec_o);
+                            o[0] = fan_q[0]; o[1] = fan_q[1]; o[2] = fan_q[2]; o[3] = fan_q[3];
+                            odd_q0 = fan_q[0]; odd_q1.x = fan_q[1].x; odd_q1.y = fan_q[1].y; odd_q3 = fan_q[3];
+                        }
+                    }
                 }
             } else {
                 if (!wireframe) {
@@ -396,12 +418,13 @@
         } else {
             *reinterpret_cast<ulonglong2*>(slot_tb + slot) = make_ulonglong2(tbs[0], tbs[3]);
             *reinterpret_cast<uint16_t*>(want + slot) = (uint16_t)(wnt[0] | (wnt[3] << 8));
-        }
-    }
-
-    {
-        __shared__ float4 s_rec[SWR_GEOM_BLOCK / 64][256];
-        static_assert(sizeof(s_rec) + 16 <= SWR_FRONT_MAX_LDS, "k_setup must fit beside the raster kernel (swr_device.h)");
+            cnt_tb0 = tbs[0]; cnt_tb1 = tbs[3]; cnt_want = wnt[0] | (wnt[3] << 8);
+        }
+    }
+
+    __shared__ float4 s_rec[SWR_GEOM_BLOCK / 64][256];
+    static_assert(sizeof(s_rec) + 16 <= SWR_FRONT_MAX_LDS, "k_setup must fit beside the raster kernel (swr_device.h)");
+    {
         const uint32_t wv = threadIdx.x >> 6, lane = threadIdx.x & 63u;
         const unsigned long long vmask = __ballot(rec_valid);
         if (vmask) {
@@ -417,6 +440,18 @@
                 if ((vmask >> j) & 1ull) dst[4u * (size_t)rec_index(slot0 + 2u * j, odd_base) + (e & 3u)] = sw[e];
             }
         }
+    }
+    if (tile_count) {
+        static_assert(sizeof(s_rec) >= 2 * SWR_BIN_TABLE * sizeof(uint32_t), "the count's hash table borrows the record staging area");
+        uint32_t* s_key = reinterpret_cast<uint32_t*>(&s_rec[0][0]);
+        uint32_t* s_val = s_key + SWR_BIN_TABLE;
+        BinArgs a;
+        a.band = band_map(fp);
+        a.tiles_x = fp.tiles_x; a.width = fp.width; a.height = fp.height;
+        a.tile_count = tile_count;
+        const uint32_t slot = 2u * (dp->tri_base + local);
+        bin_block_slots<false, SWR_GEOM_BLOCK>(a, slot_data(a.band, cnt_tb0, rec_q[0], rec_q[1], rec_q[3]), slot, cnt_want & 0xffu, s_key, s_val);
+        bin_block_slots<false, SWR_GEOM_BLOCK>(a, slot_data(a.band, cnt_tb1, odd_q0, odd_q1, odd_q3), slot + 1u, cnt_want >> 8, s_key, s_val);
     }
     __shared__ unsigned s_cnt[3];
     if (threadIdx.x < 3) s_cnt[threadIdx.x] = 0;
diff --git a/softwarerenderer_amd/csrc/swr_host.h b/softwarerenderer_amd/csrc/swr_host.h
--- a/softwarerenderer_amd/csrc/swr_host.h
+++ b/softwarerenderer_amd/csrc/swr_host.h
@@ -128,6 +128,7 @@
     std::vector<Batch> inflight;
     uint32_t next_seq = 1;
     bool sync_flush = false;
+    unsigned long long debug_max_pairs = 0;
     uint32_t debug_fill_capacity = 0;
 
     DevBuf d_slot_tb;
```

After: 78500 Mfragments/s (median of 4 runs). Within noise of the previous version (+0.1%).
